# itz-sayak/C-Users-Sayakdutta-Self-Supervised-Arbitrary-Scale-Point-Cloud-Upsampling-via-SNN

Hardware: AMD Instinct MI355X
Metric: upsampled query-points/sec (kNN + fn fwd + rotate + fd fwd + displace), 4x scale, M=48 T=4 (higher is better)
Workload: dtype f32 (GEMMs as 3 x f16 MFMA with f32 accumulation; outer kNN f64); 1 GPU; synthetic sphere N=5000 (seed 0), B=4096 grid queries per GPU per step, M=48, T=4, fn k=[24,18,12] emb 640, fd k=32 scales [8,16,32,48] emb 768, conditioned-random weights seed 0, in-patch kNN recomputed every batch; cloud_points=5000, neighbours=48, outer_knn=f64 brute force, parallelism=query shards x1

## Files before the change

c-users-sayakdutta-self-supervised-arbitrary-scale-point-cloud-upsampling-via-snn_amd/_lib.py:

```python
import ctypes
import os
from ctypes import POINTER, c_char_p, c_double, c_float, c_int, c_int32, c_int64, c_void_p

_HERE = os.path.dirname(os.path.abspath(__file__))
LIB_PATH = os.environ.get("SAPCU_LIB_PATH") or os.path.join(_HERE, "csrc", "libsapcu_hip.so")
EXACT_LIB_PATH = os.path.join(_HERE, "csrc", "libsapcu_hip_exact.so")

FN_TAPS = ("stem", "block1", "block2", "block3", "pooled", "enc", "logits")
FD_TAPS = ("fused0", "spikes", "knn", "pooled", "enc", "x0")
KIND_FN, KIND_FD = 0, 1
ABI_VERSION = 2


class SapcuLibraryError(RuntimeError):
    """The HIP library is absent or unloadable (never silently replaced by a CPU path)."""


class SapcuError(RuntimeError):
    """A C entry point returned a non-zero status: args = (code, text)."""


_SIGNATURES = {
    "sapcu_abi_version": (c_int, []),
    "sapcu_last_error": (c_char_p, []),
    "sapcu_knn_gather_f64": (c_int, [c_void_p, c_int64, c_void_p, c_int64, c_int, c_void_p, c_void_p, c_void_p, c_void_p]),
    "sapcu_gather_rotate_f64": (c_int, [c_void_p, c_int64, c_void_p, c_int64, c_void_p, c_int, c_void_p, c_void_p, c_void_p]),
    "sapcu_displace_f64": (c_int, [c_void_p, c_void_p, c_void_p, c_int64, c_void_p, c_void_p]),
    "sapcu_knn_grid_workspace_bytes": (c_int64, [c_int64]),
    "sapcu_knn_self_grid_f64": (c_int, [c_void_p, c_int64, c_int64, c_int64, c_int, c_double, c_void_p, c_void_p, c_void_p, c_int64,
                                        POINTER(c_int64), c_void_p]),
    "sapcu_outlier_stats_f64": (c_int, [c_void_p, c_int64, c_int, c_int64, c_void_p, c_void_p, c_void_p]),
    "sapcu_outlier_keep_f64": (c_int, [c_void_p, c_int64, c_double, c_double, c_void_p, c_void_p]),
    "sapcu_fps_workspace_bytes": (c_int64, [c_int64]),
    "sapcu_fps_f32": (c_int, [c_void_p, c_int64, c_int64, c_void_p, c_void_p, c_int64, c_void_p]),
    "sapcu_dense_seeds_host": (c_int, [c_void_p, c_int64, c_double, c_void_p, c_int64, POINTER(c_int64)]),
    "sapcu_lif_train_forward": (c_int, [c_void_p, c_int64, c_int, c_int] + [c_void_p] * 4 + [c_void_p, c_void_p]),
    "sapcu_lif_train_workspace_bytes": (c_int64, [c_int64, c_int]),
    "sapcu_lif_train_backward": (c_int, [c_void_p, c_void_p, c_int64, c_int, c_int] + [c_void_p] * 4 + [c_void_p] * 5 +
                                 [c_void_p, c_int64, c_void_p]),
    "sapcu_train_workspace_bytes": (c_int64, [c_int64, c_int, c_int]),
    "sapcu_bn_train_forward": (c_int, [c_void_p, c_int64, c_int, c_void_p, c_void_p, c_float] + [c_void_p] * 4 + [c_void_p, c_int64, c_void_p]),
    "sapcu_bn_train_backward": (c_int, [c_void_p, c_void_p, c_int64, c_int] + [c_void_p] * 3 + [c_void_p] * 3 + [c_void_p, c_int64, c_void_p]),
    "sapcu_conv1x1_wgrad_f32": (c_int, [c_void_p, c_int, c_void_p, c_int, c_int64, c_int, c_int, c_void_p, c_void_p, c_void_p, c_int64, c_void_p]),
    "sapcu_gemm_bf16": (c_int, [c_void_p, c_int64, c_int, c_int, c_void_p, c_int, c_void_p, c_void_p, c_int, c_void_p]),
    "sapcu_wgrad_bf16_workspace_bytes": (c_int64, [c_int64, c_int, c_int]),
    "sapcu_conv1x1_wgrad_bf16": (c_int, [c_void_p, c_int, c_void_p, c_int, c_int64, c_int, c_int, c_void_p, c_void_p, c_void_p, c_int64, c_void_p]),
    "sapcu_softmax_agg_forward": (c_int, [c_void_p, c_void_p, c_void_p, c_int, c_void_p, c_void_p, c_int64, c_int, c_int, c_int, c_float, c_void_p, c_void_p]),
    "sapcu_softmax_agg_backward": (c_int, [c_void_p, c_void_p, c_void_p, c_int, c_void_p, c_void_p, c_void_p, c_int64, c_int, c_int, c_int, c_float,
                                          c_void_p, c_void_p, c_void_p, c_int, c_void_p]),
    "sapcu_gather_rows": (c_int, [c_void_p, c_int, c_void_p, c_int64, c_int, c_void_p, c_void_p]),
    "sapcu_scatter_add_rows": (c_int, [c_void_p, c_void_p, c_int64, c_int, c_void_p, c_int, c_int64, c_void_p]),
    "sapcu_scatter_add_rows_grouped": (c_int, [c_void_p, c_void_p, c_int64, c_int, c_void_p, c_int, c_int64, c_int, c_int, c_void_p, c_void_p]),
    "sapcu_group_max_forward": (c_int, [c_void_p, c_int64, c_int, c_int, c_void_p, c_void_p, c_void_p]),
    "sapcu_group_max_backward": (c_int, [c_void_p, c_void_p, c_int64, c_int, c_int, c_void_p, c_void_p]),
    "sapcu_neuron_selfloop": (c_int, [c_void_p, c_int64, c_int, c_int] + [c_void_p] * 6 + [c_void_p] * 4 + [c_void_p]),
    "sapcu_neuron_drive": (c_int, [c_void_p, c_int64, c_int, c_int] + [c_void_p] * 6 + [c_int] + [c_void_p] * 5 + [c_void_p]),
    "sapcu_patch_knn": (c_int, [c_void_p, c_int64, c_int, c_int, c_int, c_int, c_void_p, c_void_p]),
    "sapcu_model_create": (c_int, [c_int, POINTER(c_int32), c_int, c_void_p, c_int64, POINTER(c_int64), c_int,
                                   POINTER(c_void_p)]),
    "sapcu_model_destroy": (c_int, [c_void_p]),
    "sapcu_workspace_bytes": (c_int64, [c_void_p, c_int64, c_int]),
    "sapcu_model_gate_violations": (c_int, [c_void_p, POINTER(c_int)]),
    "sapcu_l2_normalize3": (c_int, [c_void_p, c_void_p, c_int64, c_void_p]),
    "sapcu_fn_forward": (c_int, [c_void_p, c_void_p, c_int64, c_int, c_void_p, c_void_p, c_void_p, c_void_p, c_int64,
                                 POINTER(c_void_p), c_void_p]),
    "sapcu_fd_forward": (c_int, [c_void_p, c_void_p, c_int64, c_int, c_void_p, c_void_p, c_void_p, c_int64,
                                 POINTER(c_void_p), c_void_p]),
    "sapcu_gemm_f32": (c_int, [c_void_p, c_int64, c_int, c_int, c_void_p, c_int, c_void_p, c_void_p, c_int, c_void_p,
                               c_int, c_void_p, c_int, c_int, c_void_p]),
    "sapcu_to_split_rows": (c_int, [c_void_p, c_int64, c_int, c_int, c_void_p, c_int, c_void_p]),
    "sapcu_posenc_gemm_f32": (c_int, [c_void_p, c_int64, c_int, c_void_p, c_void_p, c_void_p, c_int, c_void_p, c_void_p,
                                      c_int, c_int, c_void_p, c_void_p, c_void_p, c_void_p, c_int, c_void_p]),
    "sapcu_model_gemm_mode": (c_int, [c_void_p, POINTER(c_int), POINTER(c_int)]),
    "sapcu_model_fused_blocks": (c_int, [c_void_p, c_int, POINTER(c_int)]),
    "sapcu_fn_edge_chain_workspace_bytes": (c_int64, [c_int64, c_int, c_int]),
    "sapcu_fn_edge_chain_f32": (c_int, [c_void_p, c_void_p, c_int64, c_int, c_int, c_int] + [c_void_p] * 12 + [c_int, c_int, c_void_p, c_void_p,
                                        c_int64, c_void_p]),
}

EXPORTS = tuple(_SIGNATURES)

_SEEDS_SIGNATURES = {
    "sapcu_dense_seeds_workspace_bytes": (c_int64, [c_int64, c_int64]),
    "sapcu_dense_seeds_f64": (c_int, [c_void_p, c_int64, c_double, c_void_p, c_int64, c_int64, POINTER(c_int64), POINTER(c_int64),
                              c_void_p, c_int64, c_void_p]),
}
SEEDS_EXPORTS = tuple(_SEEDS_SIGNATURES)

_INTERNAL_SIGNATURES = {
    "sapcu_internal_fold_affine_host": (c_int, [c_void_p, c_void_p, c_void_p, c_void_p, c_int, c_int, c_void_p, c_void_p]),
}
_lib = None


def load(path=None):
    global _lib
    if _lib is not None and path is None:
        return _lib
    p = path or LIB_PATH
    if not os.path.exists(p):
        raise SapcuLibraryError(
            "HIP library not built: %s is missing. Run `make -C %s` (needs hipcc, gfx950). "
            "There is no CPU fallback." % (p, os.path.dirname(p)))
    try:
        lib = ctypes.CDLL(p)
    except OSError as e:
        raise SapcuLibraryError("cannot load %s: %s" % (p, e)) from e
    for name, (res, args) in list(_SIGNATURES.items()) + list(_SEEDS_SIGNATURES.items()) + list(_INTERNAL_SIGNATURES.items()):
        try:
            fn = getattr(lib, name)
        except AttributeError as e:
            raise SapcuLibraryError("%s does not export %s" % (p, name)) from e
        fn.restype = res
        fn.argtypes = args
    if lib.sapcu_abi_version() != ABI_VERSION:
        raise SapcuLibraryError("ABI version mismatch: library %d, binding %d" % (lib.sapcu_abi_version(), ABI_VERSION))
    if path is None:
        _lib = lib
    return lib


def check(rc):
    if rc != 0:
        text = load().sapcu_last_error()
        raise SapcuError(int(rc), text.decode("utf-8", "replace") if text else "")


def ptr(t):
    return None if t is None else c_void_p(t.data_ptr())


def current_stream():
    import torch
    return c_void_p(torch.cuda.current_stream().cuda_stream)
```

c-users-sayakdutta-self-supervised-arbitrary-scale-point-cloud-upsampling-via-snn_amd/csrc/gemm_epi.h:

```cpp
#pragma once
#include "common.h"

namespace sapcu {

typedef float f32x16 __attribute__((ext_vector_type(16)));

typedef _Float16 epi_half8 __attribute__((ext_vector_type(8)));
typedef float epi_f32x4 __attribute__((ext_vector_type(4)));
__device__ __forceinline__ f32x16 mfma_32x32x16_f16(epi_half8 a, epi_half8 b, f32x16 c) {
#ifdef SAPCU_TIMING_MFMA16
    epi_f32x4 q0 = {c[0], c[1], c[2], c[3]}, q1 = {c[8], c[9], c[10], c[11]};
    q0 = __builtin_amdgcn_mfma_f32_16x16x32_f16(a, b, q0, 0, 0, 0);
    q1 = __builtin_amdgcn_mfma_f32_16x16x32_f16(a, b, q1, 0, 0, 0);
    c[0] = q0[0]; c[1] = q0[1]; c[2] = q0[2]; c[3] = q0[3];
    c[8] = q1[0]; c[9] = q1[1]; c[10] = q1[2]; c[11] = q1[3];
    return c;
#else
    return __builtin_amdgcn_mfma_f32_32x32x16_f16(a, b, c, 0, 0, 0);
#endif
}

__device__ __forceinline__ float4 ld4(const float* p) { return *reinterpret_cast<const float4*>(p); }

__device__ __forceinline__ void lds_barrier() { asm volatile("s_waitcnt lgkmcnt(0)\n\ts_barrier" ::: "memory"); }

__device__ __forceinline__ float settle(float x) {
    asm volatile("" : "+v"(x));
    return x;
}

__device__ __forceinline__ void settle4(float4& v) { asm volatile("" : "+v"(v.x), "+v"(v.y), "+v"(v.z), "+v"(v.w)); }

__device__ __forceinline__ bool split_interleaved(int ld) { return (ld & 31) == 0; }
__device__ __forceinline__ int split_hi_index(int ld, int col) { return split_interleaved(ld) ? ((col >> 5) << 6) + (col & 31) : col; }
__device__ __forceinline__ int split_lo_index(int ld, int col) { return split_interleaved(ld) ? ((col >> 5) << 6) + 32 + (col & 31) : ld + col; }

__device__ __forceinline__ void store_split(float* base, int64_t row, int ld, int col, float v) {
    _Float16* rp = reinterpret_cast<_Float16*>(base + row * ld);
    const _Float16 hi = (_Float16)v;
    rp[split_hi_index(ld, col)] = hi;
    rp[split_lo_index(ld, col)] = (_Float16)(v - (float)hi);
}

template <int EPI, int W>
__device__ __forceinline__ void epilogue_group(const GemmArgs& g, const float (&acc)[W], int64_t row, int col,
                                               float bias, const NeuronP& np, const float (&q)[W],
                                               const float (&kf)[W]) {
    float v[W], res[W];
    bool ok[W];
#pragma unroll
    for (int u = 0; u < W; ++u) ok[u] = (row + u) < g.r;
    if (EPI == EPI_RESID || EPI == EPI_RESID_GELU) {
#pragma unroll
        for (int u = 0; u < W; ++u) res[u] = ok[u] ? g.resid[(row + u) * g.ldr + col] : 0.f;
    }
#pragma unroll
    for (int u = 0; u < W; ++u) v[u] = __fadd_rn(acc[u], bias);
    if (EPI == EPI_LIF || EPI == EPI_LIF_ATTN || EPI == EPI_LIF_MAX) lif_selfloop_n<W>(v, np, g.lif_T);
#pragma unroll
    for (int u = 0; u < W; ++u) {
        if (EPI == EPI_GELU) v[u] = gelu_erf(v[u]);
        if (EPI == EPI_LRELU || EPI == EPI_LRELU_MAX) v[u] = lrelu02(v[u]);
        if (EPI == EPI_RESID) v[u] = __fadd_rn(v[u], res[u]);
        if (EPI == EPI_RESID_GELU) v[u] = gelu_erf(__fadd_rn(v[u], res[u]));
    }
    if (EPI == EPI_LRELU_MAX || EPI == EPI_LIF_MAX) {
        int64_t cur = -1;
        float best = 0.f;
#pragma unroll
        for (int u = 0; u < W; ++u) {
            if (!ok[u]) continue;
            const int64_t grp = (row + u) / g.max_m;
            if (grp != cur) {
                if (cur >= 0) atomicMax(g.max_keys + cur * g.n + col, float_max_key(best));
                cur = grp;
                best = v[u];
            } else {
                best = fmaxf(best, v[u]);
            }
        }
        if (cur >= 0) atomicMax(g.max_keys + cur * g.n + col, float_max_key(best));
        return;
    }
#pragma unroll
    for (int u = 0; u < W; ++u) {
        if (!ok[u]) continue;
        if (g.c_split) {
            store_split(g.c, row + u, g.ldc, col, v[u]);
            if (EPI != EPI_LIF && EPI != EPI_LIF_ATTN && !(fabsf(v[u]) < 65504.0f) && g.ovf) atomicAdd(g.ovf, 1);
        } else {
            g.c[(row + u) * g.ldc + col] = v[u];
        }
        if (EPI == EPI_LIF_ATTN) {
            const float ai = __fadd_rn(__fsub_rn(q[u], kf[u]), v[u]);
            if (g.c2_split) store_split(g.c2, row + u, g.ldc, col, ai);
            else g.c2[(row + u) * g.ldc + col] = ai;
        }
    }
}

struct ColParams4 {
    float4 bias;
    float4 decay, adapt, rdecay, theta0;
};

template <bool VEC>
__device__ __forceinline__ float4 ld4_cols(const float* p, int col, int n) {
    if (VEC) return ld4(p + col);
    float4 r;
    r.x = col < n ? p[col] : 0.f;
    r.y = col + 1 < n ? p[col + 1] : 0.f;
    r.z = col + 2 < n ? p[col + 2] : 0.f;
    r.w = col + 3 < n ? p[col + 3] : 0.f;
    return r;
}

template <int EPI, bool VEC>
__device__ __forceinline__ ColParams4 load_col_params4(const GemmArgs& g, int col, bool valid) {
    ColParams4 c;
    const float4 z = make_float4(0.f, 0.f, 0.f, 0.f);
    c.bias = (valid && g.bias) ? ld4_cols<VEC>(g.bias, col, g.n) : z;
    c.decay = c.adapt = c.rdecay = c.theta0 = z;
    if (EPI == EPI_LIF || EPI == EPI_LIF_ATTN) {
        const int cc = valid ? col : 0;
        c.decay = ld4_cols<VEC>(g.lif, cc, g.n);
        c.adapt = ld4_cols<VEC>(g.lif + g.n, cc, g.n);
        c.rdecay = ld4_cols<VEC>(g.lif + 2 * (int64_t)g.n, cc, g.n);
        c.theta0 = ld4_cols<VEC>(g.lif + 3 * (int64_t)g.n, cc, g.n);
    }
    return c;
}

__device__ __forceinline__ void clamp_col_params4(const ColParams4& c, NeuronP2 (&np)[2]) {
    np[0].decay = f32x2{clampf(c.decay.x, 0.1f, 0.99f), clampf(c.decay.y, 0.1f, 0.99f)};
    np[1].decay = f32x2{clampf(c.decay.z, 0.1f, 0.99f), clampf(c.decay.w, 0.1f, 0.99f)};
    np[0].adapt = f32x2{clampf(c.adapt.x, 0.001f, 0.1f), clampf(c.adapt.y, 0.001f, 0.1f)};
    np[1].adapt = f32x2{clampf(c.adapt.z, 0.001f, 0.1f), clampf(c.adapt.w, 0.001f, 0.1f)};
    np[0].rdecay = f32x2{clampf(c.rdecay.x, 0.1f, 0.95f), clampf(c.rdecay.y, 0.1f, 0.95f)};
    np[1].rdecay = f32x2{clampf(c.rdecay.z, 0.1f, 0.95f), clampf(c.rdecay.w, 0.1f, 0.95f)};
    np[0].theta0 = f32x2{c.theta0.x, c.theta0.y};
    np[1].theta0 = f32x2{c.theta0.z, c.theta0.w};
}

typedef _Float16 half4 __attribute__((ext_vector_type(4)));

template <bool VEC>
__device__ __forceinline__ void store_f32x4(float* base, int64_t row, int ld, int col, int n, const float (&v)[4]) {
    if (VEC) {
        *reinterpret_cast<float4*>(base + row * ld + col) = make_float4(v[0], v[1], v[2], v[3]);
    } else {
#pragma unroll
        for (int u = 0; u < 4; ++u)
            if (col + u < n) base[row * ld + col + u] = v[u];
    }
}

template <bool VEC>
__device__ __forceinline__ void store_split4(float* base, int64_t row, int ld, int col, int n, const float (&v)[4]) {
    if (!VEC) {
#pragma unroll
        for (int u = 0; u < 4; ++u)
            if (col + u < n) store_split(base, row, ld, col + u, v[u]);
        return;
    }
    _Float16* rp = reinterpret_cast<_Float16*>(base + row * ld);
    half4 hi, lo;
#pragma unroll
    for (int u = 0; u < 4; ++u) {
        hi[u] = (_Float16)v[u];
        lo[u] = (_Float16)(v[u] - (float)hi[u]);
    }
    *reinterpret_cast<half4*>(rp + split_hi_index(ld, col)) = hi;
    *reinterpret_cast<half4*>(rp + split_lo_index(ld, col)) = lo;
}

template <int EPI, bool VEC>
__device__ __forceinline__ void epilogue_row4_compute(const GemmArgs& g, const float4 acc, int64_t row, int col,
                                                      const ColParams4& cp, float (&v)[4]) {
    v[0] = __fmaf_rn(acc.x, 0.0625f, cp.bias.x);
    v[1] = __fmaf_rn(acc.y, 0.0625f, cp.bias.y);
    v[2] = __fmaf_rn(acc.z, 0.0625f, cp.bias.z);
    v[3] = __fmaf_rn(acc.w, 0.0625f, cp.bias.w);
    float4 res = make_float4(0.f, 0.f, 0.f, 0.f);
    if (EPI == EPI_RESID || EPI == EPI_RESID_GELU) res = ld4_cols<VEC>(g.resid + row * g.ldr, col, g.n);
    if (EPI == EPI_LIF || EPI == EPI_LIF_ATTN) {
        f32x2 pv[2] = {f32x2{v[0], v[1]}, f32x2{v[2], v[3]}};
        NeuronP2 np[2];
        clamp_col_params4(cp, np);
        lif_selfloop_pairs<2>(pv, np, g.lif_T);
        v[0] = pv[0].x; v[1] = pv[0].y; v[2] = pv[1].x; v[3] = pv[1].y;
    }
    const float rs[4] = {res.x, res.y, res.z, res.w};
#pragma unroll
    for (int u = 0; u < 4; ++u) {
        if (EPI == EPI_GELU) v[u] = gelu_erf(v[u]);
        if (EPI == EPI_LRELU) v[u] = lrelu02(v[u]);
        if (EPI == EPI_RESID) v[u] = __fadd_rn(v[u], rs[u]);
        if (EPI == EPI_RESID_GELU) v[u] = gelu_erf(__fadd_rn(v[u], rs[u]));
    }
}

template <int EPI, bool VEC>
__device__ __forceinline__ void epilogue_row4_store(const GemmArgs& g, const float (&v)[4], int64_t row, int col,
                                                    const float4 q, const float4 kf) {
    float ai[4] = {0.f, 0.f, 0.f, 0.f};
    if (EPI == EPI_LIF_ATTN) {
        ai[0] = __fadd_rn(__fsub_rn(q.x, kf.x), v[0]);
        ai[1] = __fadd_rn(__fsub_rn(q.y, kf.y), v[1]);
        ai[2] = __fadd_rn(__fsub_rn(q.z, kf.z), v[2]);
        ai[3] = __fadd_rn(__fsub_rn(q.w, kf.w), v[3]);
        asm volatile("" : "+v"(ai[0]), "+v"(ai[1]), "+v"(ai[2]), "+v"(ai[3])::"memory");
    }
    if (g.c_split) {
        store_split4<VEC>(g.c, row, g.ldc, col, g.n, v);
        if (EPI != EPI_LIF && EPI != EPI_LIF_ATTN && g.ovf) {
            float big = 0.f;
#pragma unroll
            for (int u = 0; u < 4; ++u)
                if (VEC || col + u < g.n) big = fmaxf(big, fabsf(v[u]));
            const bool nan = (VEC || col < g.n) && !(v[0] == v[0] && v[1] == v[1] && v[2] == v[2] && v[3] == v[3]);
            if (!(big < 65504.0f) || nan) atomicAdd(g.ovf, 1);
        }
    } else {
        store_f32x4<VEC>(g.c, row, g.ldc, col, g.n, v);
    }
    if (EPI == EPI_LIF_ATTN) {
        if (g.c2_split) store_split4<VEC>(g.c2, row, g.ldc, col, g.n, ai);
        else store_f32x4<VEC>(g.c2, row, g.ldc, col, g.n, ai);
    }
}

template <int EPI>
__device__ __forceinline__ void epilogue_group4(const GemmArgs& g, const float (&acc)[4], int64_t row, int col,
                                                float bias, const NeuronP& np, const float (&q)[4],
                                                const float (&kf)[4]) {
    epilogue_group<EPI, 4>(g, acc, row, col, bias, np, q, kf);
}

}
```

c-users-sayakdutta-self-supervised-arbitrary-scale-point-cloud-upsampling-via-snn_amd/csrc/gemm_f32.hip:

```cpp
#include "common.h"
#include "gemm_epi.h"

namespace sapcu {

constexpr int BM = 128, BN = 128, BK = 32, LDT = BK + 4;
constexpr int OPER_FLOATS = 2 * (BM + BN) * LDT;
constexpr int STAGE_FLOATS = 4 * 64 * 64;
constexpr int LDS_BYTES = (OPER_FLOATS + STAGE_FLOATS) * 4;

template <int EPI>
__global__ __launch_bounds__(512, 2) void gemm_kernel(const GemmArgs g) {
    extern __shared__ __attribute__((aligned(16))) float smem[];
    float* stage = smem + OPER_FLOATS;
    const int tid = threadIdx.x;
    const int lane = tid & 63, wave = tid >> 6;
    const bool producer = wave < 4;
    const int pw = wave & 3;
    const int wm = pw >> 1, wn = pw & 1;
    const int r32 = lane & 31, h = lane >> 5;

    const int ntn = (g.n + BN - 1) / BN;
    const int64_t ntm = (g.r + BM - 1) / BM;
    const int64_t ntiles = ntm * ntn;
    const int nx = gridDim.x < 8 ? 1 : 8;
// ... 57 lines not shown
            for (int i = 0; i < 4; ++i) {
                *reinterpret_cast<float4*>(&sA[(srow + 32 * i) * LDT + skc]) = ra[i];
                *reinterpret_cast<float4*>(&sW[(srow + 32 * i) * LDT + skc]) = rw[i];
            }
        };

        const bool cons_work = !producer && prev_row0 >= 0;
        float cbias[2];
        NeuronP cnp[2];
        bool ccol[2];
        if (cons_work) {
#pragma unroll
            for (int j = 0; j < 2; ++j) {
                const int col = prev_col0 + wn * 64 + j * 32 + r32;
                ccol[j] = col < g.n;
                cbias[j] = settle((ccol[j] && g.bias) ? g.bias[col] : 0.f);
                if (EPI == EPI_LIF || EPI == EPI_LIF_ATTN) {
                    cnp[j] = load_lif(g.lif, g.n, ccol[j] ? col : 0);
                    cnp[j].theta0 = settle(cnp[j].theta0);
                }
            }
        }
        const int gper = (16 + nk - 1) / nk;
        int2 tabrow = make_int2(0, 0);
        float nq[4] = {0.f, 0.f, 0.f, 0.f}, nkf[4] = {0.f, 0.f, 0.f, 0.f};
        auto issue_gather = [&](int gi) {
            if (EPI != EPI_LIF_ATTN) return;
            const int t4 = gi >> 2, e4 = gi & 3;
            const int i = t4 >> 1, j = t4 & 1;
            const int col = prev_col0 + wn * 64 + j * 32 + r32;
            const int lrow = i * 32 + 8 * e4 + 4 * h;
#pragma unroll
            for (int u = 0; u < 4; ++u) {
                const int qr = __shfl(tabrow.x, lrow + u);
                const int kr = __shfl(tabrow.y, lrow + u);
                const bool ok = col < g.n && (prev_row0 + wm * 64 + lrow + u) < g.r;
                nq[u] = ok ? g.q[(int64_t)qr * g.ldq + col] : 0.f;
                nkf[u] = ok ? g.kf[(int64_t)kr * g.ldq + col] : 0.f;
            }
        };
        if (cons_work && EPI == EPI_LIF_ATTN) {
            const int64_t trow = prev_row0 + wm * 64 + lane;
            if (trow < g.r) tabrow = g.tab[trow];
            tabrow.x = __builtin_bit_cast(int, settle(__builtin_bit_cast(float, tabrow.x)));
            tabrow.y = __builtin_bit_cast(int, settle(__builtin_bit_cast(float, tabrow.y)));
            issue_gather(0);
        }
        auto consume = [&](int s) {
            if (!cons_work) return;
            for (int gi = s * gper; gi < (s + 1) * gper && gi < 16; ++gi) {
                const int t4 = gi >> 2, e4 = gi & 3;
                const int i = t4 >> 1, j = t4 & 1;
                float cq[4], ckf[4];
#pragma unroll
                for (int u = 0; u < 4; ++u) {
                    cq[u] = nq[u];
                    ckf[u] = nkf[u];
                }
                if (gi + 1 < 16) issue_gather(gi + 1);
                if (!(j ? ccol[1] : ccol[0])) continue;
                const int64_t row = prev_row0 + wm * 64 + i * 32 + 8 * e4 + 4 * h;
                if (row >= g.r) continue;
                float a[4];
#pragma unroll
                for (int u = 0; u < 4; ++u) a[u] = stage[(pw * 64 + gi * 4 + u) * 64 + lane];
                NeuronP np;
                np.decay = j ? cnp[1].decay : cnp[0].decay;
                np.adapt = j ? cnp[1].adapt : cnp[0].adapt;
                np.rdecay = j ? cnp[1].rdecay : cnp[0].rdecay;
                np.theta0 = j ? cnp[1].theta0 : cnp[0].theta0;
                np.dT = 0.f;
                np.rh = 0.f;
                epilogue_group4<EPI>(g, a, row, prev_col0 + wn * 64 + j * 32 + r32, j ? cbias[1] : cbias[0], np, cq, ckf);
            }
        };

        if (producer && have) {
            load_tile(0);
            store_tile(0);
        }
        lds_barrier();
        int cur = 0;
        for (int kt = 0; kt < nk; ++kt) {
            if (producer) {
                if (have) {
                    if (kt + 1 < nk) load_tile((kt + 1) * BK);
                    const float* sA = smem + cur * (BM + BN) * LDT + (wm * 64 + r32) * LDT + h * 4;
                    const float* sW = smem + cur * (BM + BN) * LDT + BM * LDT + (wn * 64 + r32) * LDT + h * 4;
                    float4 fa[2][2], fb[2][2];
                    fa[0][0] = ld4(sA);
                    fa[0][1] = ld4(sA + 32 * LDT);
                    fb[0][0] = ld4(sW);
                    fb[0][1] = ld4(sW + 32 * LDT);
#pragma unroll
                    for (int k8 = 0; k8 < BK / 8; ++k8) {
                        const int cb = k8 & 1, nb = cb ^ 1;
                        if (k8 + 1 < BK / 8) {
                            fa[nb][0] = ld4(sA + (k8 + 1) * 8);
                            fa[nb][1] = ld4(sA + 32 * LDT + (k8 + 1) * 8);
                            fb[nb][0] = ld4(sW + (k8 + 1) * 8);
                            fb[nb][1] = ld4(sW + 32 * LDT + (k8 + 1) * 8);
                        }
                        const float av[2][4] = {{fa[cb][0].x, fa[cb][0].y, fa[cb][0].z, fa[cb][0].w},
                                                {fa[cb][1].x, fa[cb][1].y, fa[cb][1].z, fa[cb][1].w}};
                        const float bv[2][4] = {{fb[cb][0].x, fb[cb][0].y, fb[cb][0].z, fb[cb][0].w},
                                                {fb[cb][1].x, fb[cb][1].y, fb[cb][1].z, fb[cb][1].w}};
#pragma unroll
                        for (int e = 0; e < 4; ++e)
#pragma unroll
                            for (int i = 0; i < 2; ++i)
#pragma unroll
                                for (int j = 0; j < 2; ++j)
                                    acc[i][j] = __builtin_amdgcn_mfma_f32_32x32x2f32(av[i][e], bv[j][e], acc[i][j], 0, 0, 0);
                    }
                    if (kt + 1 < nk) store_tile(cur ^ 1);
                }
            } else {
                consume(kt);
            }
            lds_barrier();
            cur ^= 1;
        }
        if (producer && have) {
#pragma unroll
            for (int i = 0; i < 2; ++i)
#pragma unroll
                for (int j = 0; j < 2; ++j)
#pragma unroll
                    for (int e = 0; e < 16; ++e) stage[(pw * 64 + (i * 2 + j) * 16 + e) * 64 + lane] = acc[i][j][e];
        }
        lds_barrier();
        prev_row0 = have ? row0 : -1;
        prev_col0 = col0;
    }
}

template <int EPI>
static int launch_t(const GemmArgs& g, hipStream_t st) {
    static DeviceOnce lds_once;
    SAPCU_SET_MAX_LDS(lds_once, (&gemm_kernel<EPI>), LDS_BYTES);
    const int g_num_cus = device_cu_count();
    const int64_t tiles = ((g.r + BM - 1) / BM) * ((g.n + BN - 1) / BN);
    const int64_t grid = tiles < g_num_cus ? tiles : g_num_cus;
    hipLaunchKernelGGL((gemm_kernel<EPI>), dim3((unsigned)grid), dim3(512), LDS_BYTES, st, g);
    SAPCU_CHECK_LAUNCH();
    return SAPCU_OK;
}

int launch_gemm(const GemmArgs& g, hipStream_t st) {
    if (g.r == 0 || g.n == 0) return SAPCU_OK;
    SAPCU_CHECK_ARG(g.k > 0 && g.k % BK == 0, "gemm: k=%d must be a positive multiple of %d", g.k, BK);
    SAPCU_CHECK_ARG(g.lda % 4 == 0 && ((uintptr_t)g.a & 15) == 0 && ((uintptr_t)g.w & 15) == 0,
                    "gemm: A/W must be 16-byte aligned with lda %% 4 == 0 (lda=%d)", g.lda);
    switch (g.epi) {
        case EPI_BIAS: return launch_t<EPI_BIAS>(g, st);
        case EPI_LIF: return launch_t<EPI_LIF>(g, st);
        case EPI_GELU: return launch_t<EPI_GELU>(g, st);
        case EPI_RESID: return launch_t<EPI_RESID>(g, st);
        case EPI_LRELU: return launch_t<EPI_LRELU>(g, st);
        case EPI_RESID_GELU: return launch_t<EPI_RESID_GELU>(g, st);
        case EPI_LIF_ATTN:
            SAPCU_CHECK_ARG(g.ldq > 0 && g.tab && g.q && g.kf && g.c2, "gemm: bad attn operands");
            return launch_t<EPI_LIF_ATTN>(g, st);
        default: set_error("gemm: unknown epilogue %d", g.epi); return SAPCU_ERR_ARG;
    }
}

}
```

c-users-sayakdutta-self-supervised-arbitrary-scale-point-cloud-upsampling-via-snn_amd/csrc/gemm_sf16.hip:

```cpp
#include "common.h"
#include "gemm_epi.h"

namespace sapcu {

typedef _Float16 half8 __attribute__((ext_vector_type(8)));
typedef __attribute__((address_space(3))) unsigned char lds_byte;
typedef const __attribute__((address_space(1))) void* gptr_t;

constexpr int SBM = 128, SBN = 128, SBK = 64;
constexpr int PLANE_BYTES = SBM * SBK * 2;
constexpr int STAGE_BYTES = 4 * PLANE_BYTES;
constexpr int HALF_HANDOFF_BYTES = 8 * 16 * 64 * 4;
constexpr int SF16_LDS_BYTES = 2 * STAGE_BYTES + HALF_HANDOFF_BYTES;

__device__ __forceinline__ void split8(const float4& x0, const float4& x1, half8& hi, half8& lo, float& amax) {
    const float xs[8] = {x0.x, x0.y, x0.z, x0.w, x1.x, x1.y, x1.z, x1.w};
#pragma unroll
    for (int i = 0; i < 8; ++i) {
        const _Float16 h = (_Float16)xs[i];
        hi[i] = h;
        lo[i] = (_Float16)(xs[i] - (float)h);
        amax = fmaxf(amax, fabsf(xs[i]));
    }
}
// ... 134 lines not shown
                            __builtin_amdgcn_sched_barrier(0);
                        };
                        product(1, 0);
                        product(0, 1);
                        product(0, 0);
                    }
                    if (kt + 1 < nk) {
                        store_a(cur ^ 1);
                        asm volatile("s_waitcnt vmcnt(0)" ::: "memory");
                    }
                }
                lds_barrier();
                cur ^= 1;
            }
            if (have) {
#pragma unroll
                for (int e = 0; e < 16; ++e) {
                    stage0[(pw * 16 + e) * 64 + lane] = __fmul_rn(acc[0][e], 0.0625f);
                    stage1[(pw * 16 + e) * 64 + lane] = __fmul_rn(acc[1][e], 0.0625f);
                }
                if (amax > 65504.0f && g.ovf) atomicAdd(g.ovf, 1);
            }
            lds_barrier();
            prev = have;
        }
    } else {
        int64_t prev_row0 = -1;
        int prev_col0 = 0;
        const int gper = (8 + nk - 1) / nk;
        for (int64_t it = 0;; ++it) {
            const int64_t local = it * wgs_per_x + wg_in_x;
            const bool have = local < x_count;
            if (!have && prev_row0 < 0) break;
            const int64_t logical = x_begin + local;
            const bool cons_work = prev_row0 >= 0;
            float cacc[16];
#pragma unroll
            for (int q = 0; q < 16; ++q) cacc[q] = cons_work ? stage1[(pw * 16 + q) * 64 + lane] : 0.f;
            float cbias[2];
            NeuronP cnp[2];
            bool ccol[2];
#pragma unroll
            for (int j = 0; j < 2; ++j) {
                const int col = prev_col0 + wn * 64 + j * 32 + r32;
                ccol[j] = cons_work && col < g.n;
                cbias[j] = settle((ccol[j] && g.bias) ? g.bias[col] : 0.f);
                cnp[j] = NeuronP{0.f, 0.f, 0.f, 0.f, 0.f, 0.f};
                if (EPI == EPI_LIF || EPI == EPI_LIF_ATTN || EPI == EPI_LIF_MAX) {
                    cnp[j] = load_lif(g.lif, g.n, ccol[j] ? col : 0);
                    cnp[j].theta0 = settle(cnp[j].theta0);
                }
            }
            int2 tabrow = make_int2(0, 0);
            float nq[4] = {0.f, 0.f, 0.f, 0.f}, nkf[4] = {0.f, 0.f, 0.f, 0.f};
            auto issue_gather = [&](int gi) {
                if (EPI != EPI_LIF_ATTN) return;
                const int j = gi >> 2, e4 = gi & 3;
                const int col = prev_col0 + wn * 64 + j * 32 + r32;
                const int lrow = 8 * e4 + 4 * h;
#pragma unroll
                for (int u = 0; u < 4; ++u) {
                    const int qr = __shfl(tabrow.x, lrow + u);
                    const int kr = __shfl(tabrow.y, lrow + u);
                    const bool ok = col < g.n && (prev_row0 + wm * 32 + lrow + u) < g.r;
                    nq[u] = ok ? g.q[(int64_t)qr * g.ldq + col] : 0.f;
                    nkf[u] = ok ? g.kf[(int64_t)kr * g.ldq + col] : 0.f;
                }
            };
            if (cons_work && EPI == EPI_LIF_ATTN) {
                const int64_t trow = prev_row0 + wm * 32 + (lane & 31);
                if (trow < g.r) tabrow = g.tab[trow];
                tabrow.x = __builtin_bit_cast(int, settle(__builtin_bit_cast(float, tabrow.x)));
                tabrow.y = __builtin_bit_cast(int, settle(__builtin_bit_cast(float, tabrow.y)));
                issue_gather(0);
            }
            lds_barrier();
            for (int kt = 0; kt < nk; ++kt) {
                if (cons_work) {
                    for (int gi = kt * gper; gi < (kt + 1) * gper && gi < 8; ++gi) {
                        float cq[4], ckf[4];
#pragma unroll
                        for (int u = 0; u < 4; ++u) {
                            cq[u] = nq[u];
                            ckf[u] = nkf[u];
                        }
                        if (gi + 1 < 8) issue_gather(gi + 1);
                        const int j = gi >> 2, e4 = gi & 3;
                        if (!(j ? ccol[1] : ccol[0])) continue;
                        const int64_t row = prev_row0 + wm * 32 + 8 * e4 + 4 * h;
                        if (row >= g.r) continue;
                        const int col = prev_col0 + wn * 64 + j * 32 + r32;
                        if (gi < 4) {
                            float a[4];
#pragma unroll
                            for (int u = 0; u < 4; ++u) a[u] = stage0[(pw * 16 + gi * 4 + u) * 64 + lane];
                            epilogue_group4<EPI>(g, a, row, col, cbias[0], cnp[0], cq, ckf);
                        } else {
                            switch (gi) {
                                case 4: consume_reg_group<EPI, 0>(g, cacc, row, col, cbias[1], cnp[1], cq, ckf); break;
                                case 5: consume_reg_group<EPI, 1>(g, cacc, row, col, cbias[1], cnp[1], cq, ckf); break;
                                case 6: consume_reg_group<EPI, 2>(g, cacc, row, col, cbias[1], cnp[1], cq, ckf); break;
                                default: consume_reg_group<EPI, 3>(g, cacc, row, col, cbias[1], cnp[1], cq, ckf); break;
                            }
                        }
                    }
                }
                lds_barrier();
            }
            lds_barrier();
            prev_row0 = have ? (logical / ntn) * SBM : -1;
            prev_col0 = have ? (int)(logical % ntn) * SBN : 0;
        }
    }
}

__global__ __launch_bounds__(256) void split_weights_kernel(const float* __restrict__ w, int64_t count,
                                                            _Float16* __restrict__ hi, _Float16* __restrict__ lo,
                                                            int* __restrict__ ovf) {
    const int64_t t = (int64_t)blockIdx.x * blockDim.x + threadIdx.x;
    if (t >= count) return;
    const float x = w[t] * 16.0f;
    const _Float16 hh = (_Float16)x;
    hi[t] = hh;
    lo[t] = (_Float16)(x - (float)hh);
    if (!(fabsf(x) < 65504.0f)) atomicAdd(ovf, 1);
}

int launch_split_weights(const float* w, int64_t count, void* hi, void* lo, int* ovf, hipStream_t st) {
    if (count == 0) return SAPCU_OK;
    hipLaunchKernelGGL(split_weights_kernel, dim3((unsigned)((count + 255) / 256)), dim3(256), 0, st, w, count,
                       (_Float16*)hi, (_Float16*)lo, ovf);
    SAPCU_CHECK_LAUNCH();
    return SAPCU_OK;
}

template <int EPI>
static int launch_t16(const GemmArgs& g, hipStream_t st) {
    static DeviceOnce lds_once;
    SAPCU_SET_MAX_LDS(lds_once, (&gemm_sf16_kernel<EPI>), SF16_LDS_BYTES);
    const int g_num_cus16 = device_cu_count();
    const int64_t tiles = ((g.r + SBM - 1) / SBM) * ((g.n + SBN - 1) / SBN);
    const int64_t grid = tiles < g_num_cus16 ? tiles : g_num_cus16;
    hipLaunchKernelGGL((gemm_sf16_kernel<EPI>), dim3((unsigned)grid), dim3(1024), SF16_LDS_BYTES, st, g);
    SAPCU_CHECK_LAUNCH();
    return SAPCU_OK;
}

int launch_gemm_sf16(const GemmArgs& g, hipStream_t st) {
    if (g.r == 0 || g.n == 0) return SAPCU_OK;
    SAPCU_CHECK_ARG(g.k > 0 && g.k % SBK == 0, "gemm_sf16: k=%d must be a positive multiple of %d", g.k, SBK);
    SAPCU_CHECK_ARG(g.lda % 4 == 0 && ((uintptr_t)g.a & 15) == 0 && g.w16_hi && g.w16_lo &&
                        ((uintptr_t)g.w16_hi & 15) == 0 && ((uintptr_t)g.w16_lo & 15) == 0,
                    "gemm_sf16: operands must be 16-byte aligned (lda=%d)", g.lda);
    switch (g.epi) {
        case EPI_BIAS: return launch_t16<EPI_BIAS>(g, st);
        case EPI_LIF: return launch_t16<EPI_LIF>(g, st);
        case EPI_GELU: return launch_t16<EPI_GELU>(g, st);
        case EPI_RESID: return launch_t16<EPI_RESID>(g, st);
        case EPI_LRELU: return launch_t16<EPI_LRELU>(g, st);
        case EPI_LRELU_MAX:
            SAPCU_CHECK_ARG(g.max_keys && g.max_m >= 1, "gemm_sf16: EPI_LRELU_MAX needs max_keys and max_m");
            return launch_t16<EPI_LRELU_MAX>(g, st);
        case EPI_LIF_MAX:
            SAPCU_CHECK_ARG(g.max_keys && g.max_m >= 1 && g.lif, "gemm_sf16: EPI_LIF_MAX needs max_keys, max_m and neuron parameters");
            return launch_t16<EPI_LIF_MAX>(g, st);
        case EPI_RESID_GELU: return launch_t16<EPI_RESID_GELU>(g, st);
        case EPI_LIF_ATTN:
            SAPCU_CHECK_ARG(g.ldq > 0 && g.tab && g.q && g.kf && g.c2, "gemm_sf16: bad attn operands");
            return launch_t16<EPI_LIF_ATTN>(g, st);
        default: set_error("gemm_sf16: unknown epilogue %d", g.epi); return SAPCU_ERR_ARG;
    }
}

}
```

c-users-sayakdutta-self-supervised-arbitrary-scale-point-cloud-upsampling-via-snn_amd/csrc/gemm_sf16_bt.hip:

```cpp
#include "common.h"
#include "gemm_epi.h"

namespace sapcu {

typedef _Float16 half8 __attribute__((ext_vector_type(8)));
typedef __attribute__((address_space(3))) unsigned char lds_byte;
typedef const __attribute__((address_space(1))) void* gptr_t;

constexpr int TBM = 256, TBK = 32;
constexpr int TA_PLANE = TBM * TBK * 2;
constexpr int TA_SLOT = 2 * TA_PLANE;
constexpr int TA_SLOTS = 3;
constexpr int TW_SLOTS = 2;

template <int N>
__device__ __forceinline__ void bt_wait_vm() {
    if (N == 16) asm volatile("s_waitcnt vmcnt(16)" ::: "memory");
    else if (N == 8) asm volatile("s_waitcnt vmcnt(8)" ::: "memory");
    else if (N == 4) asm volatile("s_waitcnt vmcnt(4)" ::: "memory");
    else asm volatile("s_waitcnt vmcnt(0)" ::: "memory");
}

__device__ __forceinline__ float bt_load_f32(const float* p) {
    float v;
// ... 124 lines not shown
    const int kstep_bytes = a_il ? 128 : TBK * 2;
    const char* const op_base = is_a ? reinterpret_cast<const char*>(g.a) : reinterpret_cast<const char*>(g.w16_hi);
    const int pieces = is_a ? 4 : W_PIECES;
    const int rows_per_wave = 16 * pieces;
    const int depth = is_a ? TA_SLOTS : TW_SLOTS;
    const int slot_bytes = is_a ? TA_SLOT : W_SLOT;
    const int plane_bytes = is_a ? TA_PLANE : W_PLANE;
    const int64_t total_steps = my_tiles * nk;
    int64_t pf_tile = 0, pf_tm = first_tm;
    int pf_kt = 0, pf_tn = first_tn;
    const char* pf_base = nullptr;
    unsigned pf_off[4] = {0, 0, 0, 0};
    const int lrow = rows_per_wave * sub + (lane >> 2);
    auto pf_setup = [&]() {
        const int64_t first = is_a ? pf_tm * TBM : (int64_t)pf_tn * BN;
        const int64_t left = (is_a ? g.r : (int64_t)g.n) - first;
        pf_base = op_base + first * pitch_b;
#pragma unroll
        for (int p = 0; p < 4; ++p) {
            int rr = lrow + 16 * p;
            if (rr >= left) rr = (int)(left - 1);
            pf_off[p] = (unsigned)(rr * (int)pitch_b + dsb);
        }
    };
    lds_byte* const ring0 = (lds_byte*)(smem_raw + (is_a ? 0 : A_BYTES) + sub * rows_per_wave * 64);
    int issue_slot = 0;
    int64_t issued = 0;
    auto issue = [&]() {
        lds_byte* sb = ring0 + issue_slot * slot_bytes;
        const char* src = pf_base + pf_kt * kstep_bytes;
#pragma unroll
        for (int p = 0; p < 4; ++p) {
            if (p < pieces) {
                __builtin_amdgcn_global_load_lds((gptr_t)(src + pf_off[p]), sb + p * 1024, 16, 0, 0);
                __builtin_amdgcn_global_load_lds((gptr_t)(src + lo_delta + pf_off[p]), sb + plane_bytes + p * 1024, 16, 0, 0);
            }
        }
        ++issued;
        if (++issue_slot == depth) issue_slot = 0;
        if (++pf_kt == nk) {
            pf_kt = 0;
            ++pf_tile;
            pf_tm += step_tm;
            pf_tn += step_tn;
            if (pf_tn >= ntn) { pf_tn -= ntn; ++pf_tm; }
            if (pf_tile < my_tiles) pf_setup();
        }
    };
    pf_setup();
    while (issued < depth && issued < total_steps) issue();
    int64_t landed_upto = 0;
    auto wait_landed = [&](int64_t step) {
        if (step < landed_upto) return;
        const int64_t ahead = issued - step - 1;
        if (is_a) {
            if (ahead >= 2) bt_wait_vm<16>();
            else if (ahead == 1) bt_wait_vm<8>();
            else bt_wait_vm<0>();
        } else if (W_PIECES == 4) {
            if (ahead >= 1) bt_wait_vm<8>();
            else bt_wait_vm<0>();
        } else {
            if (ahead >= 1) bt_wait_vm<4>();
            else bt_wait_vm<0>();
        }
    };

    constexpr int CS = 2 * CT;
    const int c16 = lane & 15, g4 = lane >> 4;
    const unsigned frag_ko = (unsigned)((g4 ^ ((c16 >> 2) & 3)) * 16);
    const unsigned a_frag0 = (unsigned)((wm * 128 + c16) * (TBK * 2)) + frag_ko;
    const unsigned w_frag0 = (unsigned)(A_BYTES + (wn * 32 * CT + c16) * (TBK * 2)) + frag_ko;
    half8 ah0[4], al0[4], ah1[4], al1[4], wh[CS], wl[CS];
    auto read_a = [&](int a_slot, int half, half8 (&ah)[4], half8 (&al)[4]) {
        const unsigned char* sA = smem_raw + a_slot * TA_SLOT + a_frag0 + half * 4 * 16 * (TBK * 2);
#pragma unroll
        for (int i = 0; i < 4; ++i) {
            ah[i] = *reinterpret_cast<const half8*>(sA + i * 16 * (TBK * 2));
            al[i] = *reinterpret_cast<const half8*>(sA + i * 16 * (TBK * 2) + TA_PLANE);
        }
    };
    auto read_w = [&](int w_slot, int chalf) {
        const unsigned char* sW = smem_raw + w_slot * W_SLOT + w_frag0;
#pragma unroll
        for (int j = chalf * CT; j < (chalf + 1) * CT; ++j) {
            wh[j] = *reinterpret_cast<const half8*>(sW + j * 16 * (TBK * 2));
            wl[j] = *reinterpret_cast<const half8*>(sW + j * 16 * (TBK * 2) + W_PLANE);
        }
    };
    f32x4 acc[8][CS];
    auto mfma_group = [&](int rhalf, const half8 (&ah)[4], const half8 (&al)[4], int chalf) {
#pragma unroll
        for (int i = 0; i < 4; ++i)
#pragma unroll
            for (int j = chalf * CT; j < (chalf + 1) * CT; ++j)
                acc[4 * rhalf + i][j] = __builtin_amdgcn_mfma_f32_16x16x32_f16(al[i], wh[j], acc[4 * rhalf + i][j], 0, 0, 0);
#pragma unroll
        for (int i = 0; i < 4; ++i)
#pragma unroll
            for (int j = chalf * CT; j < (chalf + 1) * CT; ++j)
                acc[4 * rhalf + i][j] = __builtin_amdgcn_mfma_f32_16x16x32_f16(ah[i], wl[j], acc[4 * rhalf + i][j], 0, 0, 0);
#pragma unroll
        for (int i = 0; i < 4; ++i)
#pragma unroll
            for (int j = chalf * CT; j < (chalf + 1) * CT; ++j)
                acc[4 * rhalf + i][j] = __builtin_amdgcn_mfma_f32_16x16x32_f16(ah[i], wh[j], acc[4 * rhalf + i][j], 0, 0, 0);
    };

    wait_landed(0);
    lds_barrier();
    int ca = 0, cw = 0, na = 1, nw = 1;
    int64_t gstep = 0;
    int64_t tm = first_tm;
    int tn = first_tn;
    for (int64_t ti = 0; ti < my_tiles; ++ti) {
#pragma unroll
        for (int i = 0; i < 8; ++i)
#pragma unroll
            for (int j = 0; j < CS; ++j) acc[i][j] = f32x4{0.f, 0.f, 0.f, 0.f};
        read_w(cw, 0);
        read_w(cw, 1);
        read_a(ca, 0, ah0, al0);
        for (int kt = 0; kt < nk; ++kt, ++gstep) {
            read_a(ca, 1, ah1, al1);
            mfma_group(0, ah0, al0, 0);
            mfma_group(0, ah0, al0, 1);
            const bool more = kt + 1 < nk;
            if (gstep + 1 < total_steps) {
                wait_landed(gstep + 1);
                lds_barrier();
                if (issued < total_steps && !(is_a && kt + 1 == nk)) issue();
                if (more) read_a(na, 0, ah0, al0);
            } else {
                lds_barrier();
            }
            mfma_group(1, ah1, al1, 0);
            if (more) read_w(nw, 0);
            mfma_group(1, ah1, al1, 1);
            if (more) read_w(nw, 1);
            ca = na;
            cw = nw;
            if (++na == TA_SLOTS) na = 0;
            if (++nw == TW_SLOTS) nw = 0;
        }
        const int64_t row0 = tm * TBM + wm * 128;
        const int col0 = tn * BN + wn * 32 * CT;
        float pbias[CS], praw[CS][4];
        NeuronP pnp[CS];
#pragma unroll
        for (int j = 0; j < CS; ++j) {
            const int col = col0 + j * 16 + c16;
            pbias[j] = 0.f;
            if (g.bias) pbias[j] = bt_load_f32(g.bias + col);
            if (EPI == EPI_LIF || EPI == EPI_LIF_ATTN) {
#pragma unroll
                for (int q = 0; q < 4; ++q) praw[j][q] = bt_load_f32(g.lif + (int64_t)q * g.n + col);
            }
        }
        bt_wait_vm<0>();
        landed_upto = issued;
        if (is_a && issued < total_steps) issue();
        __builtin_amdgcn_sched_barrier(0);
#pragma unroll
        for (int j = 0; j < CS; ++j) {
            pnp[j] = NeuronP{0.f, 0.f, 0.f, 0.f, 0.f, 0.f};
            if (EPI == EPI_LIF || EPI == EPI_LIF_ATTN) {
                pnp[j].decay = clampf(praw[j][0], 0.1f, 0.99f);
                pnp[j].adapt = clampf(praw[j][1], 0.001f, 0.1f);
                pnp[j].rdecay = clampf(praw[j][2], 0.1f, 0.95f);
                pnp[j].theta0 = praw[j][3];
            }
        }
        const bool interior = tm * TBM + TBM <= g.r;
        if (EPI == EPI_LRELU_MAX) {
#pragma unroll
            for (int j = 0; j < CS; ++j) {
                const int col = col0 + j * 16 + c16;
                int64_t cur = -1, boundary = 0;
                float best = 0.f;
#pragma unroll
                for (int rs = 0; rs < 8; ++rs) {
#pragma unroll
                    for (int e = 0; e < 4; ++e) {
                        const int64_t rr = row0 + rs * 16 + 4 * g4 + e;
                        if (rr >= g.r) continue;
                        const float v = lrelu02(__fadd_rn(__fmul_rn(acc[rs][j][e], 0.0625f), pbias[j]));
                        if (rr >= boundary) {
                            if (cur >= 0) atomicMax(g.max_keys + cur * g.n + col, float_max_key(best));
                            cur = rr / g.max_m;
                            boundary = (cur + 1) * g.max_m;
                            best = v;
                        } else {
                            best = fmaxf(best, v);
                        }
                    }
                }
                if (cur >= 0) atomicMax(g.max_keys + cur * g.n + col, float_max_key(best));
            }
        } else if (interior && EPI == EPI_LIF_ATTN && !g.c_split && g.c2_split) {
            bt_epilogue_fast<EPI, CS, false, true>(g, acc, row0, col0, c16, g4, pbias, pnp);
        } else if (interior && EPI == EPI_LIF && g.c_split) {
            bt_epilogue_fast<EPI, CS, true, false>(g, acc, row0, col0, c16, g4, pbias, pnp);
        } else if (interior && EPI != EPI_LIF_ATTN && !g.c_split) {
            bt_epilogue_fast<EPI, CS, false, false>(g, acc, row0, col0, c16, g4, pbias, pnp);
        } else
#pragma unroll
        for (int rs = 0; rs < 8; ++rs) {
            const int64_t row = row0 + rs * 16 + 4 * g4;
            if (row >= g.r) continue;
            int2 t4[4];
            if (EPI == EPI_LIF_ATTN) {
#pragma unroll
                for (int u = 0; u < 4; ++u) t4[u] = row + u < g.r ? g.tab[row + u] : make_int2(0, 0);
            }
#pragma unroll
            for (int j = 0; j < CS; ++j) {
                const int col = col0 + j * 16 + c16;
                float a4[4], cq[4] = {0.f, 0.f, 0.f, 0.f}, ckf[4] = {0.f, 0.f, 0.f, 0.f};
#pragma unroll
                for (int u = 0; u < 4; ++u) a4[u] = __fmul_rn(acc[rs][j][u], 0.0625f);
                if (EPI == EPI_LIF_ATTN) {
#pragma unroll
                    for (int u = 0; u < 4; ++u) {
                        cq[u] = g.q[(int64_t)t4[u].x * g.ldq + col];
                        ckf[u] = g.kf[(int64_t)t4[u].y * g.ldq + col];
                    }
                }
                epilogue_group4<EPI>(g, a4, row, col, pbias[j], pnp[j], cq, ckf);
            }
            __builtin_amdgcn_sched_barrier(0);
        }
        tm += step_tm;
        tn += step_tn;
        if (tn >= ntn) { tn -= ntn; ++tm; }
    }
}

template <int EPI, int BN>
static int launch_bt_t(const GemmArgs& g, hipStream_t st) {
    constexpr int LDS = TA_SLOTS * TA_SLOT + TW_SLOTS * 2 * BN * TBK * 2;
    static DeviceOnce lds_once;
    SAPCU_SET_MAX_LDS(lds_once, (&gemm_bt_kernel<EPI, BN>), LDS);
    const int g_num_cus_bt = device_cu_count();
    const int64_t tiles = ((g.r + TBM - 1) / TBM) * (g.n / BN);
    const int64_t grid = tiles < g_num_cus_bt ? tiles : g_num_cus_bt;
    hipLaunchKernelGGL((gemm_bt_kernel<EPI, BN>), dim3((unsigned)grid), dim3(512), LDS, st, g);
    SAPCU_CHECK_LAUNCH();
    return SAPCU_OK;
}

bool gemm_sf16_bt_ok(const GemmArgs& g) {
    if (!g.a_split || !g.w16_hi || !g.w16_lo || g.k <= 0 || g.k % TBK || g.k > g.lda || g.lda % 8) return false;
    if (((uintptr_t)g.a & 15) || ((uintptr_t)g.w16_hi & 15) || ((uintptr_t)g.w16_lo & 15)) return false;
    if (g.n % 128) return false;
    if (4 * (int64_t)g.lda * TBM >= (1LL << 31)) return false;
    if (g.r < 4 * TBM) return false;
    auto al16 = [](const void* p) { return ((uintptr_t)p & 15) == 0; };
    if (g.ldc % 4 || !al16(g.c) || (g.bias && !al16(g.bias))) return false;
    if ((g.epi == EPI_LIF || g.epi == EPI_LIF_ATTN) && !al16(g.lif)) return false;
    if (g.epi == EPI_LIF_ATTN && (g.ldq % 4 || !al16(g.q) || !al16(g.kf) || !al16(g.c2))) return false;
    if (g.epi == EPI_LRELU_MAX) return g.max_keys != nullptr && g.max_m >= 1;
    return g.epi == EPI_BIAS || g.epi == EPI_LIF || g.epi == EPI_LIF_ATTN;
}

int launch_gemm_sf16_bt(const GemmArgs& g, hipStream_t st) {
    if (g.r == 0 || g.n == 0) return SAPCU_OK;
    SAPCU_CHECK_ARG(gemm_sf16_bt_ok(g), "gemm_bt: unsupported shape or epilogue");
    if (g.epi == EPI_LIF || g.epi == EPI_LIF_ATTN) SAPCU_CHECK_ARG(g.lif, "gemm_bt: missing neuron parameters");
    if (g.epi == EPI_LIF_ATTN) SAPCU_CHECK_ARG(g.ldq > 0 && g.tab && g.q && g.kf && g.c2, "gemm_bt: bad attn operands");
    const bool wide = g.n % 256 == 0;
    switch (g.epi) {
        case EPI_LRELU_MAX: return wide ? launch_bt_t<EPI_LRELU_MAX, 256>(g, st) : launch_bt_t<EPI_LRELU_MAX, 128>(g, st);
        case EPI_BIAS: return wide ? launch_bt_t<EPI_BIAS, 256>(g, st) : launch_bt_t<EPI_BIAS, 128>(g, st);
        case EPI_LIF: return wide ? launch_bt_t<EPI_LIF, 256>(g, st) : launch_bt_t<EPI_LIF, 128>(g, st);
        default: return wide ? launch_bt_t<EPI_LIF_ATTN, 256>(g, st) : launch_bt_t<EPI_LIF_ATTN, 128>(g, st);
    }
}


}
```

c-users-sayakdutta-self-supervised-arbitrary-scale-point-cloud-upsampling-via-snn_amd/csrc/gemm_sf16_ring.hip:

```cpp
#include "common.h"
#include "gemm_epi.h"

namespace sapcu {

typedef _Float16 half8 __attribute__((ext_vector_type(8)));
typedef __attribute__((address_space(3))) unsigned char lds_byte;
typedef const __attribute__((address_space(1))) void* gptr_t;

constexpr int RBM = 128, RBN = 128, RBK = 32;
constexpr bool RING_TILES_INTERLEAVED = true;
constexpr int RPLANE = RBM * RBK * 2;
constexpr int ROPSLOT = 2 * RPLANE;
constexpr int RING_SLOTS = 8;
constexpr int RING_BYTES = RING_SLOTS * ROPSLOT;
constexpr int RHAND = 8 * 16 * 64 * 4;
constexpr int RING_LDS_BYTES = RING_BYTES + RHAND;

template <int N>
__device__ __forceinline__ void wait_vm() {
    if (N >= 16) asm volatile("s_waitcnt vmcnt(16)" ::: "memory");
    else if (N == 12) asm volatile("s_waitcnt vmcnt(12)" ::: "memory");
    else if (N == 8) asm volatile("s_waitcnt vmcnt(8)" ::: "memory");
    else if (N == 4) asm volatile("s_waitcnt vmcnt(4)" ::: "memory");
    else asm volatile("s_waitcnt vmcnt(0)" ::: "memory");
// ... 165 lines not shown
                    acc[0] = mfma_32x32x16_f16(f1.al, f1.wh[0], acc[0]);
                    acc[1] = mfma_32x32x16_f16(f1.al, f1.wh[1], acc[1]);
                    acc[0] = mfma_32x32x16_f16(f0.ah, f0.wl[0], acc[0]);
                    acc[1] = mfma_32x32x16_f16(f0.ah, f0.wl[1], acc[1]);
                    acc[0] = mfma_32x32x16_f16(f1.ah, f1.wl[0], acc[0]);
                    acc[1] = mfma_32x32x16_f16(f1.ah, f1.wl[1], acc[1]);
                    acc[0] = mfma_32x32x16_f16(f0.ah, f0.wh[0], acc[0]);
                    acc[1] = mfma_32x32x16_f16(f0.ah, f0.wh[1], acc[1]);
                    acc[0] = mfma_32x32x16_f16(f1.ah, f1.wh[0], acc[0]);
                    acc[1] = mfma_32x32x16_f16(f1.ah, f1.wh[1], acc[1]);
                    if (gstep + 1 < total_steps) {
                        wait_landed(gstep + 1);
                        lds_barrier();
                        if (issued < total_steps) issue();
                        read_frags(na, nw, 0, f0);
                    } else {
                        lds_barrier();
                    }
                    ca = na;
                    cw = nw;
                    if (++na == RA_SLOTS) na = 0;
                    if (++nw == RW_SLOTS) nw = 0;
                    continue;
                }
                mfma6(f0);
                if (gstep + 1 < total_steps) {
                    wait_landed(gstep + 1);
                    lds_barrier();
                    if (issued < total_steps) issue();
                    read_frags(na, nw, 0, f0);
                } else {
                    lds_barrier();
                }
                mfma6(f1);
                ca = na;
                cw = nw;
                if (++na == RA_SLOTS) na = 0;
                if (++nw == RW_SLOTS) nw = 0;
            }
#pragma unroll
            for (int jj = 0; jj < 2; ++jj) {
                const int j = 1 - jj;
                lds_barrier();
#pragma unroll
                for (int e = 0; e < 16; ++e) {
                    float* hb = (e & 1) ? hand_odd : hand_even;
                    hb[((e & 3) + 8 * (e >> 2)) * 32] = acc[j][e];
                }
                lds_barrier();
            }
        }
    } else {
        const int c4 = lane & 7, rs = lane >> 3;
        auto hand_at = [&](int p) -> const float4* {
            const int rr = p * 8 + rs;
            return reinterpret_cast<const float4*>(hand + pw * 1024 + (rr ^ ((rr >> 2) & 1)) * 32 + c4 * 4);
        };
        float4 cacc[4];
        int64_t prev_row0 = -1;
        int prev_col0 = 0;
        int64_t cur_tm = first_tm;
        int cur_tn = first_tn;
        const int pper = (8 + nk - 1) / nk;
        lds_barrier();
        for (int64_t ti = 0; ti <= my_tiles; ++ti) {
            const bool have = ti < my_tiles;
            const bool cons_work = prev_row0 >= 0;
            bool ccol[2];
#pragma unroll
            for (int j = 0; j < 2; ++j) ccol[j] = cons_work && (prev_col0 + wn * 64 + j * 32 + c4 * 4) < g.n;
            ColParams4 cp;
            cp.bias = cp.decay = cp.adapt = cp.rdecay = cp.theta0 = make_float4(0.f, 0.f, 0.f, 0.f);
            int2 tabrow = make_int2(0, 0);
            if (cons_work && EPI == EPI_LIF_ATTN) {
                const int64_t trow = prev_row0 + wm * 32 + (lane & 31);
                if (trow < g.r) tabrow = g.tab[trow];
                tabrow.x = __builtin_bit_cast(int, settle(__builtin_bit_cast(float, tabrow.x)));
                tabrow.y = __builtin_bit_cast(int, settle(__builtin_bit_cast(float, tabrow.y)));
            }
            for (int kt = 0; kt < nk; ++kt) {
                if (cons_work)
                for (int pi = kt * pper; pi < (kt + 1) * pper && pi < 8; ++pi) {
                    const int j = pi >> 2, p4 = pi & 3, rr = p4 * 8 + rs;
                    const int64_t row = prev_row0 + wm * 32 + rr;
                    const int col = prev_col0 + wn * 64 + j * 32 + c4 * 4;
                    const bool active = (j ? ccol[1] : ccol[0]) && row < g.r;
                    if (p4 == 0) {
                        cp = load_col_params4<EPI, VEC>(g, col, j ? ccol[1] : ccol[0]);
                        settle4(cp.bias);
                        if (EPI == EPI_LIF || EPI == EPI_LIF_ATTN) {
                            settle4(cp.decay);
                            settle4(cp.adapt);
                            settle4(cp.rdecay);
                            settle4(cp.theta0);
                        }
                    }
                    float4 cq = make_float4(0.f, 0.f, 0.f, 0.f), ckf = cq;
                    if (EPI == EPI_LIF_ATTN) {
                        const int qr = __shfl(tabrow.x, rr);
                        const int kr = __shfl(tabrow.y, rr);
                        if (active) {
                            cq = ld4_cols<VEC>(g.q + (int64_t)qr * g.ldq, col, g.n);
                            ckf = ld4_cols<VEC>(g.kf + (int64_t)kr * g.ldq, col, g.n);
                        }
                    }
                    if (!active) continue;
                    float4 a;
                    if (j == 0) a = *hand_at(p4);
                    else switch (p4) {
                        case 0: a = cacc[0]; break;
                        case 1: a = cacc[1]; break;
                        case 2: a = cacc[2]; break;
                        default: a = cacc[3]; break;
                    }
                    float v[4];
                    epilogue_row4_compute<EPI, VEC>(g, a, row, col, cp, v);
                    epilogue_row4_store<EPI, VEC>(g, v, row, col, cq, ckf);
                }
                if (have) lds_barrier();
            }
            if (!have) break;
            lds_barrier();
            lds_barrier();
#pragma unroll
            for (int p = 0; p < 4; ++p) cacc[p] = *hand_at(p);
            lds_barrier();
            lds_barrier();
            prev_row0 = cur_tm * RBM;
            prev_col0 = cur_tn * RBN;
            cur_tm += step_tm;
            cur_tn += step_tn;
            if (cur_tn >= ntn) { cur_tn -= ntn; ++cur_tm; }
        }
    }
}

template <int EPI, bool VEC, bool PM = false>
static int launch_ring_tv(const GemmArgs& g, hipStream_t st) {
    static DeviceOnce lds_once;
    SAPCU_SET_MAX_LDS(lds_once, (&gemm_ring_kernel<EPI, VEC, PM>), RING_LDS_BYTES);
    const int g_num_cus_ring = device_cu_count();
    const int row_step = RBM;
    const int64_t tiles = ((g.r + row_step - 1) / row_step) * ((g.n + RBN - 1) / RBN);
    const int64_t grid = tiles < g_num_cus_ring ? tiles : g_num_cus_ring;
    hipLaunchKernelGGL((gemm_ring_kernel<EPI, VEC, PM>), dim3((unsigned)grid), dim3(1024), RING_LDS_BYTES, st, g);
    SAPCU_CHECK_LAUNCH();
    return SAPCU_OK;
}

static bool ring_vec_ok(const GemmArgs& g) {
    auto al16 = [](const void* p) { return ((uintptr_t)p & 15) == 0; };
    bool ok = g.n % 4 == 0 && g.ldc % 4 == 0 && al16(g.c) && (!g.bias || al16(g.bias));
    if (g.epi == EPI_LIF || g.epi == EPI_LIF_ATTN) ok = ok && al16(g.lif);
    if (g.epi == EPI_RESID || g.epi == EPI_RESID_GELU) ok = ok && g.ldr % 4 == 0 && al16(g.resid);
    if (g.epi == EPI_LIF_ATTN) ok = ok && g.ldq % 4 == 0 && al16(g.q) && al16(g.kf) && al16(g.c2);
    return ok;
}

template <int EPI>
static int launch_ring_t(const GemmArgs& g, hipStream_t st) {
    return ring_vec_ok(g) ? launch_ring_tv<EPI, true, true>(g, st) : launch_ring_tv<EPI, false, true>(g, st);
}
int launch_gemm_sf16_ring(const GemmArgs& g, hipStream_t st) {
    if (g.r == 0 || g.n == 0) return SAPCU_OK;
    SAPCU_CHECK_ARG(g.a_split, "gemm_ring: A must be in split rows");
    SAPCU_CHECK_ARG(g.k > 0 && g.k % RBK == 0 && g.k <= g.lda, "gemm_ring: k=%d must be a multiple of %d and <= lda", g.k, RBK);
    SAPCU_CHECK_ARG(g.lda % 8 == 0 && ((uintptr_t)g.a & 15) == 0 && g.w16_hi && g.w16_lo &&
                        ((uintptr_t)g.w16_hi & 15) == 0 && ((uintptr_t)g.w16_lo & 15) == 0,
                    "gemm_ring: operands must be 16-byte aligned with lda %% 8 == 0 (lda=%d)", g.lda);
    if (g.epi == EPI_LIF || g.epi == EPI_LIF_ATTN) SAPCU_CHECK_ARG(g.lif, "gemm_ring: missing neuron parameters");
    if (g.epi == EPI_RESID || g.epi == EPI_RESID_GELU) SAPCU_CHECK_ARG(g.resid, "gemm_ring: missing residual");
    switch (g.epi) {
        case EPI_BIAS: return launch_ring_t<EPI_BIAS>(g, st);
        case EPI_LIF: return launch_ring_t<EPI_LIF>(g, st);
        case EPI_GELU: return launch_ring_t<EPI_GELU>(g, st);
        case EPI_RESID: return launch_ring_t<EPI_RESID>(g, st);
        case EPI_LRELU: return launch_ring_t<EPI_LRELU>(g, st);
        case EPI_RESID_GELU: return launch_ring_t<EPI_RESID_GELU>(g, st);
        case EPI_LIF_ATTN:
            SAPCU_CHECK_ARG(g.ldq > 0 && g.tab && g.q && g.kf && g.c2, "gemm_ring: bad attn operands");
            return launch_ring_t<EPI_LIF_ATTN>(g, st);
        default: set_error("gemm_ring: unknown epilogue %d", g.epi); return SAPCU_ERR_ARG;
    }
}


}
```

c-users-sayakdutta-self-supervised-arbitrary-scale-point-cloud-upsampling-via-snn_amd/csrc/model.hip:

```cpp
#include <stdarg.h>
#include <stdlib.h>

#include <new>
#include <vector>

#include "common.h"
#include "ops.h"

namespace sapcu {

static thread_local char g_err[512] = "";

void set_error(const char* fmt, ...) {
    va_list ap;
    va_start(ap, fmt);
    vsnprintf(g_err, sizeof(g_err), fmt, ap);
    va_end(ap);
}

enum FnSlot {
    FN_STEM_W = 0, FN_STEM_B, FN_STEM_LIF,
    FN_BLK0 = 3,
    FN_FINAL_W = FN_BLK0 + 63, FN_FINAL_B, FN_FINAL_LIF,
    FN_FCOUT_W, FN_FCOUT_B,
    FN_MLP0_W, FN_MLP0_B, FN_MLP1_W, FN_MLP1_B, FN_MLP2_W, FN_MLP2_B,
    FN_HEAD_W, FN_HEAD_B, FN_LN_W, FN_LN_B,
    FN_SLOTS
};
enum FnBlkSlot {
    B_FC1_W = 0, B_FC1_B, B_SNN1,
    B_QKV_W, B_QKV_B, B_QKV_LIF,
    B_DELTA_W, B_DELTA_B, B_DELTA_LIF,
    B_DELTA2_W, B_DELTA2_B, B_DELTA2_LIF,
    B_GAMMA_W, B_GAMMA_B, B_GAMMA_LIF,
    B_GAMMA2_W, B_GAMMA2_B,
    B_OUT_W, B_OUT_B,
    B_FC2_W, B_FC2_B,
    B_SLOTS
};
static_assert(B_SLOTS == 21, "fn block slot count");
static_assert(FN_SLOTS == 81, "fn slot count");

enum FdSlot {
    FD_E0_W = 0, FD_E0_B,
    FD_FUSE_W, FD_FUSE_B, FD_SNN0,
    FD_EDGE1_W, FD_EDGE1_SHIFT, FD_SNN1,
    FD_EDGE2_W, FD_EDGE2_SHIFT, FD_SNN2,
    FD_EDGE3_W, FD_EDGE3_SHIFT, FD_SNN3,
    FD_MSC_W, FD_MSC_B,
    FD_TI_W, FD_SNNFC,
    FD_FCIN_W, FD_FCIN_B,
    FD_R0_FC0_W, FD_R0_FC0_B, FD_R0_FC4_W, FD_R0_FC4_B, FD_R0_PROJ_W, FD_R0_PROJ_B,
    FD_R1_FC0_W, FD_R1_FC0_B, FD_R1_FC4_W, FD_R1_FC4_B, FD_R1_PROJ_W, FD_R1_PROJ_B,
    FD_QKV_W, FD_QKV_B,
    FD_WO_T, FD_BO, FD_LN_W, FD_LN_B, FD_WH_T, FD_BH, FD_WD, FD_BD,
    FD_SLOTS
};
static_assert(FD_SLOTS == 42, "fd slot count");

}

struct sapcu_model {
    int kind;
    int kv[3];
    int k, nscale;
    int ks[8];
    int32_t* ks_dev;
    int* gate_dev;
    bool sf16;
    void* w16_hi;
    void* w16_lo;
    void* chain_w;
    int* ovf_dev;
    int emb, T, heads;
    int64_t chunk;
    int64_t ws_budget;
    bool opt_bt;
    bool opt_chain;
    bool opt_chain_wide;
    bool opt_fn_maxfuse;
    bool opt_fn_fold_out;
    bool opt_fd_maxfuse;
    bool opt_fd_split;
    bool opt_fd_fused;
    bool opt_fd_x0;
    void* fde_w;
    int64_t fde_off[5];
    float* fde_nprm;
    float* blob;
    int64_t blob_floats;
    int64_t fold_w[3], fold_b[3];
    std::vector<int64_t> dir;
    const float* p(int slot) const { return blob + dir[slot]; }
};

namespace sapcu {

struct Arena {
    char* base;
    int64_t cap, off;
    template <typename T>
    T* take(int64_t count) {
        const int64_t bytes = ((count * (int64_t)sizeof(T)) + 255) & ~(int64_t)255;
        T* p = reinterpret_cast<T*>(base + off);
        off += bytes;
        return p;
    }
};

static inline int64_t imax(int64_t a, int64_t b) { return a > b ? a : b; }
static inline int imin(int a, int b) { return a < b ? a : b; }

static bool split_rows_gemm_on_big_tile(const GemmArgs& g, bool allow_bt) { return allow_bt && gemm_sf16_bt_ok(g); }

int launch_gemm_split_rows(const GemmArgs& g, hipStream_t st, bool allow_bt) {
    if (split_rows_gemm_on_big_tile(g, allow_bt)) return launch_gemm_sf16_bt(g, st);
    return launch_gemm_sf16_ring(g, st);
}

static void fold_affine_f64(const float* w1, const float* b1, const float* w2, const float* b2, int d, int n, float* w_fold,
                            float* b_fold) {
    std::vector<double> acc((size_t)d);
    for (int i = 0; i < n; ++i) {
        for (int k = 0; k < d; ++k) acc[k] = 0.0;
        double bs = 0.0;
        for (int j = 0; j < d; ++j) {
            const double a = (double)w2[(int64_t)i * d + j];
            const float* row = w1 + (int64_t)j * d;
            for (int k = 0; k < d; ++k) acc[k] += a * (double)row[k];
            bs += a * (double)b1[j];
        }
        for (int k = 0; k < d; ++k) w_fold[(int64_t)i * d + k] = (float)acc[k];
        b_fold[i] = (float)(bs + (double)b2[i]);
    }
}

static bool env_off(const char* name) {
    const char* e = getenv(name);
    return e && strcmp(e, "0") == 0;
}

static int run_gemm(const sapcu_model* m, GemmArgs& g, hipStream_t st) {
    const bool have16 = m && m->sf16 && g.w >= m->blob && g.w < m->blob + m->blob_floats;
    if (have16) {
        const int64_t off = g.w - m->blob;
        g.w16_hi = (const _Float16*)m->w16_hi + off;
        g.w16_lo = (const _Float16*)m->w16_lo + off;
        g.ovf = m->ovf_dev;
        if (g.a_split) return launch_gemm_split_rows(g, st, m->opt_bt);
        if (g.k % 64 == 0) return launch_gemm_sf16(g, st);
    }
    if (g.a_split || g.c_split || g.c2_split) {
        set_error("run_gemm: split-row operands need the split-f16 kernels");
        return SAPCU_ERR_ARG;
    }
    return launch_gemm(g, st);
}

static int gemm(const sapcu_model* m, const float* a, int64_t r, int k, int lda, const float* w, int n,
                const float* bias, float* c, int ldc, int epi, hipStream_t st, const float* lif = nullptr,
                int lifT = 0, const float* resid = nullptr, int ldr = 0, int fmt = 0) {
    GemmArgs g;
    memset(&g, 0, sizeof(g));
    g.a = a; g.r = r; g.k = k; g.lda = lda; g.w = w; g.n = n; g.bias = bias; g.c = c; g.ldc = ldc;
    g.epi = epi; g.lif = lif; g.lif_T = lifT; g.resid = resid; g.ldr = ldr;
    g.a_split = fmt & 1; g.c_split = (fmt >> 1) & 1;
    return run_gemm(m, g, st);
}

#define SAPCU_TRY(expr)                 \
    do {                                \
        int _rc = (expr);               \
        if (_rc != SAPCU_OK) return _rc; \
    } while (0)

static int tap_copy(void* const* taps, int which, int64_t dst_off_bytes, const void* src, int64_t bytes,
                    hipStream_t st) {
    if (!taps || !taps[which] || bytes == 0) return SAPCU_OK;
    SAPCU_CHECK_HIP(hipMemcpyAsync((char*)taps[which] + dst_off_bytes, src, (size_t)bytes, hipMemcpyDeviceToDevice, st));
    return SAPCU_OK;
}

struct FnPlan {
    int64_t cb;
    int kk[3];
    int64_t edge_floats, edge_floats23;
};

static bool fn_block_fused(const sapcu_model* m, int l, int mp) {
    return m->sf16 && m->chain_w && m->opt_chain && fn_edge_chain_ok(128 << l, imin(m->kv[l], mp));
}

static void fn_edge_floats_per_patch(const sapcu_model* m, int mp, int64_t& first, int64_t& others) {
    first = (int64_t)mp * m->emb;
    others = 0;
    for (int l = 0; l < 3; ++l) {
        if (fn_block_fused(m, l, mp)) continue;
        const int64_t e = (int64_t)mp * imin(m->kv[l], mp) * (128 << l);
        first = imax(first, e);
        others = imax(others, e);
    }
}

static int64_t fn_bytes_per_patch(const sapcu_model* m, int mp) {
    int64_t e1, e23;
    fn_edge_floats_per_patch(m, mp, e1, e23);
    int kmx = 1;
    int64_t idxs = 0;
    for (int l = 0; l < 3; ++l) {
        const int kk = imin(m->kv[l], mp);
        idxs += (int64_t)mp * kk * 4;
        kmx = kmx > kk ? kmx : kk;
    }
    return (e1 + 2 * e23) * 4 + idxs + (int64_t)mp * kmx * 24 + (int64_t)mp * (64 + 192 + 512 + 1536 + 512) * 4 +
           ((int64_t)m->emb + 2048 + 1024 + 512 + 256 + 3) * 4;
}

static int64_t chunk_patches(const sapcu_model* m, int64_t b, int64_t bytes_per_patch) {
    int64_t cb = m->chunk;
    if (cb <= 0) {
        cb = m->ws_budget / (bytes_per_patch > 0 ? bytes_per_patch : 1);
        cb = cb < 64 ? 64 : (cb / 64) * 64;
    }
    if (cb > b) cb = b;
    return cb < 1 ? 1 : cb;
}

static FnPlan fn_plan(const sapcu_model* m, int64_t b, int mp) {
    FnPlan pl;
    pl.cb = chunk_patches(m, b, fn_bytes_per_patch(m, mp));
    for (int l = 0; l < 3; ++l) pl.kk[l] = imin(m->kv[l], mp);
    int64_t e1, e23;
    fn_edge_floats_per_patch(m, mp, e1, e23);
    pl.edge_floats = e1 * pl.cb;
    pl.edge_floats23 = e23 * pl.cb;
    return pl;
}

static int64_t fn_ws_bytes(const sapcu_model* m, int64_t b, int mp) {
    const FnPlan pl = fn_plan(m, b, mp);
    const int64_t P = pl.cb * mp;
    int64_t fl = 0;
    auto add = [&](int64_t n, int64_t esz) { fl += ((n * esz) + 255) & ~(int64_t)255; };
    for (int l = 0; l < 3; ++l) add(P * pl.kk[l], 4);
    { int kmx = 1; for (int l = 0; l < 3; ++l) kmx = kmx > pl.kk[l] ? kmx : pl.kk[l]; add(P * kmx, 8); add(P * kmx, 16); }
    add(P * 64, 4); add(P * 192, 4); add(P * 512, 4); add(P * 1536, 4); add(P * 512, 4);
    add(pl.edge_floats, 4); add(pl.edge_floats23, 4); add(pl.edge_floats23, 4);
    add(pl.cb * m->emb, 4); add(pl.cb * 2048, 4); add(pl.cb * 1024, 4); add(pl.cb * 512, 4); add(pl.cb * 256, 4);
    add(pl.cb * 3, 4);
    return fl + 256;
}

static int fn_forward(const sapcu_model* m, const float* patch, int64_t b, int mp, const int32_t* knn_in,
                      int32_t* knn_out, float* normals, void* ws, int64_t ws_bytes, void* const* taps,
                      hipStream_t st) {
    const FnPlan pl = fn_plan(m, b, mp);
    if (ws_bytes < fn_ws_bytes(m, b, mp)) {
        set_error("fn_forward: workspace %lld B < required %lld B", (long long)ws_bytes, (long long)fn_ws_bytes(m, b, mp));
        return SAPCU_ERR_WORKSPACE;
    }
    int64_t tab_off[3];
    tab_off[0] = 0;
    tab_off[1] = b * mp * pl.kk[0];
    tab_off[2] = tab_off[1] + b * mp * pl.kk[1];

    for (int64_t s = 0; s < b; s += pl.cb) {
        const int64_t cb = (b - s) < pl.cb ? (b - s) : pl.cb;
        const int64_t P = cb * mp;
        Arena A{(char*)(((uintptr_t)ws + 255) & ~(uintptr_t)255), ws_bytes, 0};
        int32_t* idx[3];
        for (int l = 0; l < 3; ++l) idx[l] = A.take<int32_t>(pl.cb * mp * pl.kk[l]);
        int kmx = 1;
        for (int l = 0; l < 3; ++l) kmx = kmx > pl.kk[l] ? kmx : pl.kk[l];
        int2* tab = A.take<int2>(pl.cb * mp * kmx);
        float4* pdiff = A.take<float4>(pl.cb * mp * kmx);
        float* feat0 = A.take<float>(pl.cb * mp * 64);
        float* cat = A.take<float>(pl.cb * mp * 192);
        float* X = A.take<float>(pl.cb * mp * 512);
        float* QKV = A.take<float>(pl.cb * mp * 1536);
        float* RES = A.take<float>(pl.cb * mp * 512);
        float* B1 = A.take<float>(pl.edge_floats);
        float* B2 = A.take<float>(pl.edge_floats23);
        float* B3 = A.take<float>(pl.edge_floats23);
        float* pooled = A.take<float>(pl.cb * m->emb);
        float* enc = A.take<float>(pl.cb * 2048);
        float* h1 = A.take<float>(pl.cb * 1024);
        float* h2 = A.take<float>(pl.cb * 512);
        float* h3 = A.take<float>(pl.cb * 256);
        float* logits = A.take<float>(pl.cb * 3);
        const float* pc = patch + s * mp * 3;

        if (!knn_in) SAPCU_TRY(launch_patch_knn_multi(pc, cb, (int64_t)mp * 3, mp, 3, 3, 3, pl.kk, idx, st));
        for (int l = 0; l < 3; ++l) {
            const int64_t cnt = P * pl.kk[l];
            if (knn_in)
                SAPCU_CHECK_HIP(hipMemcpyAsync(idx[l], knn_in + tab_off[l] + s * mp * pl.kk[l], cnt * 4,
                                               hipMemcpyDeviceToDevice, st));
            if (knn_out)
                SAPCU_CHECK_HIP(hipMemcpyAsync(knn_out + tab_off[l] + s * mp * pl.kk[l], idx[l], cnt * 4,
                                               hipMemcpyDeviceToDevice, st));
        }
        SAPCU_TRY(launch_fn_stem(pc, P, m->p(FN_STEM_W), m->p(FN_STEM_B), m->p(FN_STEM_LIF), m->T, feat0, st));
        SAPCU_TRY(tap_copy(taps, SAPCU_FN_TAP_STEM, s * mp * 64 * 4, feat0, P * 64 * 4, st));

        const float* fin = feat0;
        int ldin = 64;
        for (int l = 0; l < 3; ++l) {
            const int d = 128 << l;
            const int kk = pl.kk[l];
            const int64_t R = P * kk;
            const int sb = FN_BLK0 + l * B_SLOTS;
            const int SP = m->sf16 ? 1 : 0;
            SAPCU_TRY(gemm(m, fin, P, 64, ldin, m->p(sb + B_FC1_W), d, m->p(sb + B_FC1_B), X, d, EPI_LIF, st,
                           m->p(sb + B_SNN1), 4, nullptr, 0, SP << 1));
            SAPCU_TRY(gemm(m, X, P, d, d, m->p(sb + B_QKV_W), 3 * d, m->p(sb + B_QKV_B), QKV, 3 * d, EPI_LIF, st,
                           m->p(sb + B_QKV_LIF), 4, nullptr, 0, SP));
            const float sqrt_hd = (float)sqrt((double)(d / m->heads));
            if (fn_block_fused(m, l, mp)) {
                ChainArgs ca;
                memset(&ca, 0, sizeof(ca));
                ca.P = P; ca.m = mp; ca.qkv = QKV; ca.ldq = 3 * d;
                ca.wd = m->p(sb + B_DELTA_W); ca.bd = m->p(sb + B_DELTA_B); ca.lifd = m->p(sb + B_DELTA_LIF);
                static const int64_t cw_off[3] = {0, (int64_t)3 * 2 * 128 * 128, (int64_t)3 * 2 * (128 * 128 + 256 * 256)};
                const _Float16* cw = (const _Float16*)m->chain_w + cw_off[l];
                ca.w1p = cw; ca.b1 = m->p(sb + B_DELTA2_B); ca.lif1 = m->p(sb + B_DELTA2_LIF);
                ca.w2p = cw + (int64_t)d * d * 2; ca.b2 = m->p(sb + B_GAMMA_B); ca.lif2 = m->p(sb + B_GAMMA_LIF);
                ca.w3p = cw + (int64_t)2 * d * d * 2; ca.b3 = m->p(sb + B_GAMMA2_B);
                ca.inv_sqrt_hd = 1.0f / sqrt_hd;
                ca.res = RES; ca.res_split = SP; ca.T = 4; ca.wide_offsets = m->opt_chain_wide ? 1 : 0;
                SAPCU_TRY(launch_fn_edge_chain(ca, pc, idx[l], d, kk, tab, pdiff, st));
            } else {
                SAPCU_TRY(launch_fn_pe1(pc, idx[l], R, mp, kk, d, m->p(sb + B_DELTA_W), m->p(sb + B_DELTA_B),
                                        m->p(sb + B_DELTA_LIF), 4, B1, SP, st));
                {
                    GemmArgs g;
                    memset(&g, 0, sizeof(g));
                    g.a = B1; g.r = R; g.k = d; g.lda = d; g.w = m->p(sb + B_DELTA2_W); g.n = d;
                    g.bias = m->p(sb + B_DELTA2_B); g.c = B2; g.ldc = d; g.epi = EPI_LIF_ATTN;
                    g.lif = m->p(sb + B_DELTA2_LIF); g.lif_T = 4; g.c2 = B3;
                    g.q = QKV; g.kf = QKV + d; g.ldq = 3 * d; g.tab = tab;
                    g.a_split = SP; g.c2_split = SP;
                    SAPCU_TRY(launch_edge_table(idx[l], R, mp, kk, tab, st));
                    SAPCU_TRY(run_gemm(m, g, st));
                }
                SAPCU_TRY(gemm(m, B3, R, d, d, m->p(sb + B_GAMMA_W), d, m->p(sb + B_GAMMA_B), B1, d, EPI_LIF, st,
                               m->p(sb + B_GAMMA_LIF), 4, nullptr, 0, SP | (SP << 1)));
                {
                    SAPCU_TRY(gemm(m, B1, R, d, d, m->p(sb + B_GAMMA2_W), d, m->p(sb + B_GAMMA2_B), B3, d, EPI_BIAS, st, nullptr, 0,
                                   nullptr, 0, SP));
                    SAPCU_TRY(launch_fn_softmax_agg(B3, B2, QKV + 2 * d, 3 * d, idx[l], P, mp, kk, d, sqrt_hd, RES, SP, st));
                }
            }
            if (m->opt_fn_fold_out) {
                SAPCU_TRY(gemm(m, RES, P, d, d, m->blob + m->fold_w[l], 64, m->blob + m->fold_b[l], cat + 64 * l, 192, EPI_RESID, st,
                               nullptr, 0, fin, ldin, SP));
            } else {
                SAPCU_TRY(gemm(m, RES, P, d, d, m->p(sb + B_OUT_W), d, m->p(sb + B_OUT_B), X, d, EPI_BIAS, st, nullptr, 0, nullptr,
                               0, SP | (SP << 1)));
                SAPCU_TRY(gemm(m, X, P, d, d, m->p(sb + B_FC2_W), 64, m->p(sb + B_FC2_B), cat + 64 * l, 192, EPI_RESID, st,
                               nullptr, 0, fin, ldin, SP));
            }
            if (taps && taps[SAPCU_FN_TAP_BLOCK1 + l]) {
                SAPCU_CHECK_HIP(hipMemcpy2DAsync((char*)taps[SAPCU_FN_TAP_BLOCK1 + l] + s * mp * 64 * 4, 64 * 4,
                                                 cat + 64 * l, 192 * 4, 64 * 4, (size_t)P, hipMemcpyDeviceToDevice, st));
            }
            fin = cat + 64 * l;
            ldin = 192;
        }
        if (m->sf16 && m->opt_fn_maxfuse) {
            GemmArgs g;
            memset(&g, 0, sizeof(g));
            g.a = cat; g.r = P; g.k = 192; g.lda = 192; g.w = m->p(FN_FINAL_W); g.n = m->emb; g.bias = m->p(FN_FINAL_B);
            g.ldc = m->emb; g.epi = EPI_LIF_MAX; g.lif = m->p(FN_FINAL_LIF); g.lif_T = m->T;
            g.max_keys = reinterpret_cast<unsigned*>(B1); g.max_m = mp;
            SAPCU_CHECK_HIP(hipMemsetAsync(g.max_keys, 0, (size_t)cb * m->emb * 4, st));
            SAPCU_TRY(run_gemm(m, g, st));
            SAPCU_TRY(launch_decode_max_keys(g.max_keys, cb * m->emb, pooled, st));
        } else {
            SAPCU_TRY(gemm(m, cat, P, 192, 192, m->p(FN_FINAL_W), m->emb, m->p(FN_FINAL_B), B1, m->emb, EPI_LIF, st,
                           m->p(FN_FINAL_LIF), m->T));
            SAPCU_TRY(launch_rowgroup_max(B1, cb, mp, m->emb, pooled, st));
        }
        SAPCU_TRY(tap_copy(taps, SAPCU_FN_TAP_POOLED, s * m->emb * 4, pooled, cb * m->emb * 4, st));
        SAPCU_TRY(gemm(m, pooled, cb, m->emb, m->emb, m->p(FN_FCOUT_W), 2048, m->p(FN_FCOUT_B), enc, 2048, EPI_BIAS, st));
        SAPCU_TRY(tap_copy(taps, SAPCU_FN_TAP_ENC, s * 2048 * 4, enc, cb * 2048 * 4, st));
        SAPCU_TRY(gemm(m, enc, cb, 2048, 2048, m->p(FN_MLP0_W), 1024, m->p(FN_MLP0_B), h1, 1024, EPI_GELU, st));
        SAPCU_TRY(gemm(m, h1, cb, 1024, 1024, m->p(FN_MLP1_W), 512, m->p(FN_MLP1_B), h2, 512, EPI_GELU, st));
        SAPCU_TRY(gemm(m, h2, cb, 512, 512, m->p(FN_MLP2_W), 256, m->p(FN_MLP2_B), h3, 256, EPI_GELU, st));
        SAPCU_TRY(launch_fn_tail(h3, cb, 256, m->p(FN_HEAD_W), m->p(FN_HEAD_B), m->p(FN_LN_W), m->p(FN_LN_B), logits,
                                 normals + s * 3, st));
        SAPCU_TRY(tap_copy(taps, SAPCU_FN_TAP_LOGITS, s * 3 * 4, logits, cb * 3 * 4, st));
    }
    return SAPCU_OK;
}

struct FdPlan {
    int64_t cb;
    int kmax0, kk;
    bool fused;
    bool x0path;
    bool maxfuse;
    int64_t agg_rows(int mp) const { return maxfuse ? 1 : mp; }
};

static bool fd_encoder_fused(const sapcu_model* m, int mp) {
    return m->sf16 && m->opt_fd_fused && m->fde_w && m->fde_nprm && fd_encoder_ok(mp, m->nscale, m->emb, m->T);
}

static bool fd_x0_path(const sapcu_model* m, int mp) {
    return !fd_encoder_fused(m, mp) && m->sf16 && m->opt_fd_fused && m->opt_fd_x0 && m->opt_fd_maxfuse && m->opt_fd_split && m->fde_w &&
           m->fde_nprm && fd_msc_ok(mp, m->emb, m->T);
}

static FdPlan fd_plan(const sapcu_model* m, int64_t b, int mp) {
    FdPlan pl;
    pl.fused = fd_encoder_fused(m, mp);
    pl.x0path = fd_x0_path(m, mp);
    pl.maxfuse = m->sf16 && m->opt_fd_maxfuse;
    if (pl.fused) {
        const int64_t per_patch_f = ((int64_t)(m->T + 1) * m->emb + 256 + 3 * 128 + 3 * 64 + 192 + 64) * 4;
        pl.cb = chunk_patches(m, b, per_patch_f);
        int kmaxf = 1;
        for (int i = 0; i < m->nscale; ++i) kmaxf = kmaxf > m->ks[i] ? kmaxf : m->ks[i];
        pl.kmax0 = imin(kmaxf, mp);
        pl.kk = imin(m->k, mp);
        return pl;
    }
    int kmax0 = 1;
    for (int i = 0; i < m->nscale; ++i) kmax0 = kmax0 > m->ks[i] ? kmax0 : m->ks[i];
    const int64_t slabs = pl.x0path ? 2 : m->T;
    const int64_t per_patch = (int64_t)mp * ((slabs * 960 + 960 + 1024 + 64 * (m->nscale + 1)) * 4 +
                                            (int64_t)(imin(kmax0, mp) + 3 * imin(m->k, mp)) * 4) +
                              (int64_t)m->T * pl.agg_rows(mp) * m->emb * 4 +
                              ((int64_t)(m->T + 1) * m->emb + 256 + 3 * 128 + 3 * 64 + 192 + 64) * 4;
    pl.cb = chunk_patches(m, b, per_patch);
    int kmax = 1;
    for (int i = 0; i < m->nscale; ++i) kmax = kmax > m->ks[i] ? kmax : m->ks[i];
    pl.kmax0 = imin(kmax, mp);
    pl.kk = imin(m->k, mp);
    return pl;
}

static int64_t fd_ws_bytes(const sapcu_model* m, int64_t b, int mp) {
    const FdPlan pl = fd_plan(m, b, mp);
    const int64_t P = pl.cb * mp;
    int64_t fl = 0;
    auto add = [&](int64_t n, int64_t esz) { fl += ((n * esz) + 255) & ~(int64_t)255; };
    if (!pl.fused) {
        add(P * pl.kmax0, 4); add(3 * P * pl.kk, 4);
        add(P * 64 * m->nscale, 4); add(P * 64, 4);
        add((pl.x0path ? 1 : (int64_t)m->T) * P * 960, 4); add(P * 960, 4); add(P * 1024, 4); add((int64_t)m->T * pl.cb * pl.agg_rows(mp) * m->emb, 4);
        if (pl.x0path) add(P * 960, 4);
    }
    add((int64_t)m->T * pl.cb * m->emb, 4); add(pl.cb * m->emb, 4);
    add(pl.cb * 256, 4);
    for (int i = 0; i < 3; ++i) add(pl.cb * 128, 4);
    for (int i = 0; i < 3; ++i) add(pl.cb * 64, 4);
    add(pl.cb * 192, 4); add(pl.cb * 64, 4);
    return fl + 256;
}

static int fd_forward(const sapcu_model* m, const float* patch, int64_t b, int mp, const int32_t* knn_force,
                      float* dist, void* ws, int64_t ws_bytes, void* const* taps, hipStream_t st) {
    const FdPlan pl = fd_plan(m, b, mp);
    if (ws_bytes < fd_ws_bytes(m, b, mp)) {
        set_error("fd_forward: workspace %lld B < required %lld B", (long long)ws_bytes, (long long)fd_ws_bytes(m, b, mp));
        return SAPCU_ERR_WORKSPACE;
    }
    const int T = m->T, emb = m->emb;
    static const int cin[4] = {0, 64, 128, 256}, cout[4] = {64, 128, 256, 512}, coff[4] = {0, 64, 192, 448};
    for (int64_t s = 0; s < b; s += pl.cb) {
        const int64_t cb = (b - s) < pl.cb ? (b - s) : pl.cb;
        const int64_t P = cb * mp;
        Arena A{(char*)(((uintptr_t)ws + 255) & ~(uintptr_t)255), ws_bytes, 0};
        const int64_t pp = pl.fused ? 0 : 1;
        int32_t* idx0 = A.take<int32_t>(pp * pl.cb * mp * pl.kmax0);
        int32_t* idxb = A.take<int32_t>(pp * 3 * pl.cb * mp * pl.kk);
        float* E0 = A.take<float>(pp * pl.cb * mp * 64 * m->nscale);
        float* FUSED = A.take<float>(pp * pl.cb * mp * 64);
        float* SPK = A.take<float>(pp * (pl.x0path ? 1 : (int64_t)T) * pl.cb * mp * 960);
        float* F0 = A.take<float>(pp * pl.cb * mp * 960);
        float* AB = A.take<float>(pp * pl.cb * mp * 1024);
        float* AGG = A.take<float>(pp * (int64_t)T * pl.cb * pl.agg_rows(mp) * emb);
        float* X0 = A.take<float>(pl.x0path ? pl.cb * mp * 960 : 0);
        float* POOLED = A.take<float>((int64_t)T * pl.cb * emb);
        float* ENC = A.take<float>(pl.cb * emb);
        float* D1 = A.take<float>(pl.cb * 256);
        float* D2a = A.take<float>(pl.cb * 128);
        float* D2b = A.take<float>(pl.cb * 128);
        float* D2c = A.take<float>(pl.cb * 128);
        float* D3a = A.take<float>(pl.cb * 64);
        float* D3b = A.take<float>(pl.cb * 64);
        float* D3c = A.take<float>(pl.cb * 64);
        float* QKV = A.take<float>(pl.cb * 192);
        float* ATT = A.take<float>(pl.cb * 64);
        const float* pc = patch + s * mp * 3;

        if (pl.fused) {
            FdEncArgs ea;
            memset(&ea, 0, sizeof(ea));
            ea.patch = pc; ea.b = cb; ea.b_total = b; ea.s0 = s;
            ea.m = mp; ea.T = T; ea.kk = pl.kk; ea.kmax0 = pl.kmax0; ea.nscale = m->nscale; ea.emb = emb;
            for (int i = 0; i < 4; ++i) ea.ks[i] = i < m->nscale ? imin(m->ks[i], mp) : 0;
            ea.e0_w = m->p(FD_E0_W); ea.e0_b = m->p(FD_E0_B);
            const _Float16* fw = (const _Float16*)m->fde_w;
            ea.fuse_wp = fw + m->fde_off[0]; ea.fuse_b = m->p(FD_FUSE_B);
            for (int l = 0; l < 3; ++l) {
                ea.edge_wp[l] = fw + m->fde_off[1 + l];
                ea.shift[l] = m->p(FD_EDGE1_SHIFT + 3 * l);
            }
            ea.msc_wp = fw + m->fde_off[4]; ea.msc_b = m->p(FD_MSC_B);
            ea.nprm = m->fde_nprm;
            ea.pooled = POOLED;
            ea.knn_force = knn_force;
            ea.tap_knn = taps ? (int32_t*)taps[SAPCU_FD_TAP_KNN] : nullptr;
            ea.tap_fused0 = taps ? (float*)taps[SAPCU_FD_TAP_FUSED0] : nullptr;
            ea.tap_spikes = taps ? (float*)taps[SAPCU_FD_TAP_SPIKES] : nullptr;
            ea.tap_x0 = taps ? (float*)taps[SAPCU_FD_TAP_X0] : nullptr;
            ea.gate = m->gate_dev; ea.ovf = m->ovf_dev;
            SAPCU_TRY(launch_fd_encoder(ea, st));
        } else {
        SAPCU_TRY(launch_patch_knn(pc, cb, mp, 3, 3, pl.kmax0, idx0, st));
        SAPCU_TRY(launch_fd_edge0(pc, idx0, pl.kmax0, P, mp, m->nscale, m->ks_dev, m->p(FD_E0_W), m->p(FD_E0_B), E0, st));
        SAPCU_TRY(gemm(m, E0, P, 64 * m->nscale, 64 * m->nscale, m->p(FD_FUSE_W), 64, m->p(FD_FUSE_B), FUSED, 64,
                       EPI_LRELU, st));
        SAPCU_TRY(tap_copy(taps, SAPCU_FD_TAP_FUSED0, s * mp * 64 * 4, FUSED, P * 64 * 4, st));
        float* const X0T = (taps && taps[SAPCU_FD_TAP_X0]) ? (float*)taps[SAPCU_FD_TAP_X0] + s * mp * 960 : nullptr;
        if (X0T) SAPCU_CHECK_HIP(hipMemcpy2DAsync(X0T, 960 * 4, FUSED, 64 * 4, 64 * 4, (size_t)P, hipMemcpyDeviceToDevice, st));
// ... 168 lines not shown
}

int sapcu_patch_knn(const float* feat, int64_t b, int m, int c, int ld, int k, int32_t* idx_out, void* stream) {
    SAPCU_CHECK_ARG(feat && idx_out && b >= 0 && ld >= c, "patch_knn: bad argument");
    return launch_patch_knn(feat, b, m, c, ld, k, idx_out, (hipStream_t)stream);
}

int sapcu_l2_normalize3(const float* in, float* out, int64_t b, void* stream) {
    SAPCU_CHECK_ARG(in && out && b >= 0, "l2_normalize3: bad argument");
    return launch_l2_normalize3(in, out, b, (hipStream_t)stream);
}

static int split_into_ws(const float* w, int64_t cnt, void* w16_ws, GemmArgs& g, hipStream_t st) {
    char* base = (char*)w16_ws;
    int* ovf = (int*)(base + 4 * cnt);
    SAPCU_CHECK_HIP(hipMemsetAsync(ovf, 0, sizeof(int), st));
    SAPCU_TRY(launch_split_weights(w, cnt, base, base + 2 * cnt, ovf, st));
    g.w16_hi = (const _Float16*)base;
    g.w16_lo = (const _Float16*)(base + 2 * cnt);
    g.ovf = ovf;
    return SAPCU_OK;
}

int sapcu_gemm_f32(const float* a, int64_t r, int k, int lda, const float* w, int n, const float* bias,
                   const float* lif4, int lif_steps, float* c, int ldc, void* w16_ws, int a_split_rows, int c_split_rows,
                   void* stream) {
    SAPCU_CHECK_ARG(a && w && c && r >= 0 && n >= 1, "gemm: bad argument");
    SAPCU_CHECK_ARG(!lif4 || lif_steps >= 1, "gemm: lif_steps must be >= 1");
    SAPCU_CHECK_ARG(!(a_split_rows || c_split_rows) || w16_ws, "gemm: split rows need the split-f16 kernels (w16_ws)");
    SAPCU_CHECK_ARG(r == 0 || (k > 0 && k % 32 == 0 && lda >= k && ldc >= n), "gemm: need k %% 32 == 0, lda >= k and ldc >= n (k=%d lda=%d n=%d ldc=%d)", k, lda, n, ldc);
    SAPCU_CHECK_ARG(r == 0 || ((((uintptr_t)a | (uintptr_t)w | (uintptr_t)w16_ws) & 15) == 0 && lda % (a_split_rows ? 8 : 4) == 0),
                    "gemm: A, W and w16_ws must be 16-byte aligned, lda %% 4 == 0 (%% 8 for split rows) (lda=%d)", lda);
    GemmArgs g;
    memset(&g, 0, sizeof(g));
    g.a = a; g.r = r; g.k = k; g.lda = lda; g.w = w; g.n = n; g.bias = bias; g.c = c; g.ldc = ldc;
    g.epi = lif4 ? EPI_LIF : EPI_BIAS; g.lif = lif4; g.lif_T = lif_steps;
    g.a_split = a_split_rows ? 1 : 0; g.c_split = c_split_rows ? 1 : 0;
    if (w16_ws && (g.a_split || k % 64 == 0)) {
        SAPCU_TRY(split_into_ws(w, (int64_t)n * k, w16_ws, g, (hipStream_t)stream));
        return g.a_split ? launch_gemm_split_rows(g, (hipStream_t)stream, a_split_rows != 2) : launch_gemm_sf16(g, (hipStream_t)stream);
    }
    SAPCU_CHECK_ARG(!g.c_split, "gemm: split-row output needs k %% 64 == 0 on the f32-A path");
    return launch_gemm(g, (hipStream_t)stream);
}

int sapcu_to_split_rows(const float* in, int64_t rows, int k, int ld_in, float* out, int ld_out, void* stream) {
    SAPCU_CHECK_ARG(in && out && rows >= 0 && k >= 1 && ld_in >= k && ld_out >= k, "to_split_rows: bad argument");
    return launch_to_split_rows(in, rows, k, ld_in, out, ld_out, (hipStream_t)stream);
}

int sapcu_posenc_gemm_f32(const float* pe1, int64_t r, int d, const float* w, const float* bias, const float* lif4,
                          int lif_steps, const float* qkv, const int32_t* idx, int kk, int m_pts, float* pe_out,
                          float* attn_in_out, void* edge_table_ws, void* w16_ws, int split_rows, void* stream) {
    SAPCU_CHECK_ARG(pe1 && w && lif4 && qkv && idx && pe_out && attn_in_out && edge_table_ws && r >= 0 && d >= 32 &&
                        lif_steps >= 1 && kk >= 1 && m_pts >= 1,
                    "posenc_gemm: bad argument");
    SAPCU_CHECK_ARG(!split_rows || w16_ws, "posenc_gemm: split rows need the split-f16 kernels (w16_ws)");
    SAPCU_CHECK_ARG(d % 32 == 0, "posenc_gemm: d=%d must be a multiple of 32", d);
    SAPCU_CHECK_ARG((((uintptr_t)pe1 | (uintptr_t)w | (uintptr_t)w16_ws) & 15) == 0 && ((uintptr_t)edge_table_ws & 7) == 0,
                    "posenc_gemm: pe1, w and w16_ws must be 16-byte aligned, edge_table_ws 8-byte aligned");
    GemmArgs g;
    memset(&g, 0, sizeof(g));
    g.a = pe1; g.r = r; g.k = d; g.lda = d; g.w = w; g.n = d; g.bias = bias; g.c = pe_out; g.ldc = d;
    g.epi = EPI_LIF_ATTN; g.lif = lif4; g.lif_T = lif_steps; g.c2 = attn_in_out;
    g.q = qkv; g.kf = qkv + d; g.ldq = 3 * d; g.tab = (const int2*)edge_table_ws;
    SAPCU_TRY(launch_edge_table(idx, r, m_pts, kk, (int2*)edge_table_ws, (hipStream_t)stream));
    if (w16_ws && (split_rows || d % 64 == 0)) {
        SAPCU_TRY(split_into_ws(w, (int64_t)d * d, w16_ws, g, (hipStream_t)stream));
        if (split_rows) {
            g.a_split = 1;
            g.c2_split = 1;
            return launch_gemm_split_rows(g, (hipStream_t)stream, split_rows != 2);
        }
        return launch_gemm_sf16(g, (hipStream_t)stream);
    }
    return launch_gemm(g, (hipStream_t)stream);
}

int64_t sapcu_fn_edge_chain_workspace_bytes(int64_t points, int d, int kk) {
    if (points < 0 || !fn_edge_chain_ok(d, kk)) {
        set_error("fn_edge_chain_workspace_bytes: unsupported shape (d=%d kk=%d)", d, kk);
        return SAPCU_ERR_ARG;
    }
    const int64_t rows = points * kk;
    auto up = [](int64_t b) { return (b + 255) & ~(int64_t)255; };
    return up(rows * 8) + up(rows * 16) + 3 * (up((int64_t)d * d * 4 + 16) + up((int64_t)d * d * 4)) + 256;
}

int sapcu_fn_edge_chain_f32(const float* patch, const int32_t* idx, int64_t points, int m_pts, int d, int kk,
                            const float* qkv, const float* w_delta, const float* b_delta, const float* lif_delta,
                            const float* w1, const float* b1, const float* lif1, const float* w2, const float* b2,
                            const float* lif2, const float* w3, const float* b3, int heads, int lif_steps,
                            float* res_out, void* workspace, int64_t workspace_bytes, void* stream) {
    SAPCU_CHECK_ARG(patch && idx && qkv && w_delta && b_delta && lif_delta && w1 && b1 && lif1 && w2 && b2 && lif2 && w3 && b3 &&
                        res_out && workspace, "fn_edge_chain: null pointer");
    SAPCU_CHECK_ARG(fn_edge_chain_ok(d, kk), "fn_edge_chain: unsupported shape (d=%d kk=%d)", d, kk);
    SAPCU_CHECK_ARG(points >= 0 && m_pts >= kk && heads >= 1 && d % heads == 0 && lif_steps >= 1, "fn_edge_chain: bad sizes");
    const int64_t need = sapcu_fn_edge_chain_workspace_bytes(points, d, kk);
    if (workspace_bytes < need) {
        set_error("fn_edge_chain: workspace %lld B < required %lld B", (long long)workspace_bytes, (long long)need);
        return SAPCU_ERR_WORKSPACE;
    }
    hipStream_t st = (hipStream_t)stream;
    Arena A{(char*)(((uintptr_t)workspace + 255) & ~(uintptr_t)255), workspace_bytes, 0};
    int2* tab = A.take<int2>(points * kk);
    float4* pd = A.take<float4>(points * kk);
    const float* ws[3] = {w1, w2, w3};
    const _Float16* packed[3];
    for (int q = 0; q < 3; ++q) {
        char* split = A.take<char>((int64_t)d * d * 4 + 16);
        _Float16* pk = A.take<_Float16>((int64_t)d * d * 2);
        GemmArgs g;
        memset(&g, 0, sizeof(g));
        SAPCU_TRY(split_into_ws(ws[q], (int64_t)d * d, split, g, st));
        SAPCU_TRY(launch_pack_chain_weights(g.w16_hi, g.w16_lo, d, pk, st));
        packed[q] = pk;
    }
    ChainArgs ca;
    memset(&ca, 0, sizeof(ca));
    ca.P = points; ca.m = m_pts; ca.qkv = qkv; ca.ldq = 3 * d;
    ca.wd = w_delta; ca.bd = b_delta; ca.lifd = lif_delta;
    ca.w1p = packed[0]; ca.b1 = b1; ca.lif1 = lif1;
    ca.w2p = packed[1]; ca.b2 = b2; ca.lif2 = lif2;
    ca.w3p = packed[2]; ca.b3 = b3;
    ca.inv_sqrt_hd = 1.0f / (float)sqrt((double)(d / heads));
    ca.res = res_out; ca.res_split = 0; ca.T = lif_steps;
    return launch_fn_edge_chain(ca, patch, idx, d, kk, tab, pd, st);
}

int sapcu_model_create(int kind, const int32_t* hp, int n_hp, const float* blob, int64_t blob_floats,
                       const int64_t* dir_host, int n_dir, sapcu_model_t* out) {
    SAPCU_CHECK_ARG(hp && blob && dir_host && out && blob_floats > 0, "model_create: null pointer");
    sapcu_model* m = new (std::nothrow) sapcu_model();
    SAPCU_CHECK_ARG(m != nullptr, "model_create: out of host memory");
    m->kind = kind;
    m->ks_dev = nullptr;
    m->gate_dev = nullptr;
    m->blob = nullptr;
    m->w16_hi = nullptr;
    m->w16_lo = nullptr;
    m->chain_w = nullptr;
    m->ovf_dev = nullptr;
    m->fde_w = nullptr;
    m->fde_nprm = nullptr;
    const char* ge = getenv("SAPCU_GEMM");
    m->sf16 = !(ge && strcmp(ge, "f32") == 0);
    m->opt_bt = !env_off("SAPCU_BT");
    m->opt_chain = !env_off("SAPCU_CHAIN");
    {
        const char* v = getenv("SAPCU_CHAIN");
        m->opt_chain_wide = v && strcmp(v, "wide") == 0;
    }
    m->opt_fn_maxfuse = !env_off("SAPCU_FN_MAXFUSE");
    m->opt_fn_fold_out = !env_off("SAPCU_FN_FOLD_OUT");
    for (int l = 0; l < 3; ++l) m->fold_w[l] = m->fold_b[l] = 0;
    m->opt_fd_maxfuse = !env_off("SAPCU_FD_MAXFUSE");
    m->opt_fd_split = !env_off("SAPCU_FD_SPLIT");
    m->opt_fd_fused = !env_off("SAPCU_FD_FUSED");
    m->opt_fd_x0 = !env_off("SAPCU_FD_X0");
    const char* ce = getenv("SAPCU_CHUNK");
    m->chunk = ce ? atoll(ce) : 0;
    if (m->chunk < 0) m->chunk = 0;
    const char* be = getenv("SAPCU_WS_BUDGET_MB");
    m->ws_budget = (be ? atoll(be) : 20480) * (int64_t)(1 << 20);
    if (m->ws_budget < (int64_t)(64 << 20)) m->ws_budget = (int64_t)(64 << 20);
    int rc = SAPCU_OK;
    if (kind == SAPCU_KIND_FN) {
        if (n_hp != 6 || n_dir != FN_SLOTS) {
            set_error("model_create(fn): need 6 hparams and %d slots (got %d, %d)", (int)FN_SLOTS, n_hp, n_dir);
            rc = SAPCU_ERR_ARG;
        } else {
            m->kv[0] = hp[0]; m->kv[1] = hp[1]; m->kv[2] = hp[2];
            m->emb = hp[3]; m->T = hp[4]; m->heads = hp[5];
            if (m->kv[0] < 1 || m->kv[1] < 1 || m->kv[2] < 1 || m->emb < 32 || m->emb % 32 || m->T < 1 || m->heads < 1 ||
                128 % m->heads) {
                set_error("model_create(fn): unsupported hyper-parameters");
                rc = SAPCU_ERR_ARG;
            }
        }
    } else if (kind == SAPCU_KIND_FD) {
        if (n_hp < 6 || n_dir != FD_SLOTS || hp[4] < 1 || hp[4] > 8 || n_hp != 5 + hp[4]) {
            set_error("model_create(fd): need [k,emb,T,heads,S,ks...] and %d slots", (int)FD_SLOTS);
            rc = SAPCU_ERR_ARG;
        } else {
            m->k = hp[0]; m->emb = hp[1]; m->T = hp[2]; m->heads = hp[3]; m->nscale = hp[4];
            for (int i = 0; i < m->nscale; ++i) m->ks[i] = hp[5 + i];
            if (m->k < 1 || m->emb < 32 || m->emb % 32 || m->T < 1 || m->T > 64 || m->heads < 1) {
                set_error("model_create(fd): unsupported hyper-parameters");
                rc = SAPCU_ERR_ARG;
            }
        }
    } else {
        set_error("model_create: unknown kind %d", kind);
        rc = SAPCU_ERR_ARG;
    }
    if (rc == SAPCU_OK) {
        m->dir.assign(dir_host, dir_host + n_dir);
        for (int i = 0; i < n_dir; ++i)
            if (m->dir[i] < 0 || m->dir[i] >= blob_floats || (m->dir[i] & 3)) {
                set_error("model_create: slot %d offset %lld out of range / unaligned", i, (long long)m->dir[i]);
                rc = SAPCU_ERR_ARG;
                break;
            }
    }
    auto hip_ok = [&](hipError_t e, const char* what) {
        if (e != hipSuccess && rc == SAPCU_OK) {
            set_error("model_create: %s failed: %s", what, hipGetErrorString(e));
            rc = SAPCU_ERR_HIP;
        }
    };
    if (rc == SAPCU_OK) {
        int64_t total = blob_floats;
        if (kind == SAPCU_KIND_FN && m->opt_fn_fold_out) {
            total = (total + 63) & ~(int64_t)63;
            for (int l = 0; l < 3; ++l) {
                m->fold_w[l] = total;
                total += (int64_t)64 * (128 << l);
                m->fold_b[l] = total;
                total += 64;
            }
        }
        m->blob_floats = total;
        hip_ok(hipMalloc((void**)&m->blob, (size_t)total * 4), "hipMalloc(blob)");
        if (rc == SAPCU_OK) hip_ok(hipMemcpy(m->blob, blob, (size_t)blob_floats * 4, hipMemcpyDeviceToDevice), "copy blob");
        if (rc == SAPCU_OK && total > blob_floats)
            hip_ok(hipMemset(m->blob + blob_floats, 0, (size_t)(total - blob_floats) * 4), "memset folded parameters");
        for (int l = 0; l < 3 && rc == SAPCU_OK && total > blob_floats; ++l) {
            const int d = 128 << l, sb = FN_BLK0 + l * B_SLOTS;
            const int64_t need[4] = {(int64_t)d * d, d, (int64_t)64 * d, 64};
            static const int slot[4] = {B_OUT_W, B_OUT_B, B_FC2_W, B_FC2_B};
            std::vector<float> h[4], wf((size_t)64 * d), bf(64);
            for (int q = 0; q < 4 && rc == SAPCU_OK; ++q) {
                if (m->dir[sb + slot[q]] + need[q] > blob_floats) {
                    set_error("model_create(fn): slot %d runs past the end of the blob", sb + slot[q]);
                    rc = SAPCU_ERR_ARG;
                    break;
                }
                h[q].resize((size_t)need[q]);
                hip_ok(hipMemcpy(h[q].data(), m->p(sb + slot[q]), (size_t)need[q] * 4, hipMemcpyDeviceToHost), "read out_proj / fc2");
            }
            if (rc != SAPCU_OK) break;
            fold_affine_f64(h[0].data(), h[1].data(), h[2].data(), h[3].data(), d, 64, wf.data(), bf.data());
            hip_ok(hipMemcpy(m->blob + m->fold_w[l], wf.data(), wf.size() * 4, hipMemcpyHostToDevice), "copy folded weights");
            if (rc == SAPCU_OK) hip_ok(hipMemcpy(m->blob + m->fold_b[l], bf.data(), bf.size() * 4, hipMemcpyHostToDevice), "copy folded bias");
        }
        if (rc == SAPCU_OK) hip_ok(hipMalloc((void**)&m->ovf_dev, 2 * sizeof(int)), "hipMalloc(ovf)");
        if (rc == SAPCU_OK) hip_ok(hipMemset(m->ovf_dev, 0, 2 * sizeof(int)), "memset ovf");
        if (rc == SAPCU_OK && m->sf16) {
            hip_ok(hipMalloc(&m->w16_hi, (size_t)total * 2), "hipMalloc(w16_hi)");
            if (rc == SAPCU_OK) hip_ok(hipMalloc(&m->w16_lo, (size_t)total * 2), "hipMalloc(w16_lo)");
            if (rc == SAPCU_OK) {
                int wovf = 0;
                if (launch_split_weights(m->blob, total, m->w16_hi, m->w16_lo, m->ovf_dev + 1, nullptr) != SAPCU_OK)
                    rc = SAPCU_ERR_HIP;
                if (rc == SAPCU_OK) hip_ok(hipMemcpy(&wovf, m->ovf_dev + 1, sizeof(int), hipMemcpyDeviceToHost), "read ovf");
                if (rc == SAPCU_OK && wovf != 0) m->sf16 = false;
            }
            if (rc == SAPCU_OK && m->sf16 && kind == SAPCU_KIND_FN) {
                const int64_t halves = (int64_t)3 * 2 * (128 * 128 + 256 * 256 + 512 * 512);
                hip_ok(hipMalloc(&m->chain_w, (size_t)halves * 2), "hipMalloc(chain_w)");
                int64_t off = 0;
                for (int l = 0; l < 3 && rc == SAPCU_OK; ++l) {
                    const int d = 128 << l;
                    static const int slots[3] = {B_DELTA2_W, B_GAMMA_W, B_GAMMA2_W};
                    for (int q = 0; q < 3 && rc == SAPCU_OK; ++q) {
                        const int64_t wo = m->dir[FN_BLK0 + l * B_SLOTS + slots[q]];
                        if (launch_pack_chain_weights((const _Float16*)m->w16_hi + wo, (const _Float16*)m->w16_lo + wo, d,
                                                      (_Float16*)m->chain_w + off, nullptr) != SAPCU_OK)
                            rc = SAPCU_ERR_HIP;
                        off += (int64_t)d * d * 2;
                    }
                }
                if (rc == SAPCU_OK) hip_ok(hipDeviceSynchronize(), "pack chain weights");
            }
        }
        if (rc == SAPCU_OK && kind == SAPCU_KIND_FD) {
            hip_ok(hipMalloc((void**)&m->ks_dev, 8 * sizeof(int32_t)), "hipMalloc(ks)");
            if (rc == SAPCU_OK) hip_ok(hipMemcpy(m->ks_dev, m->ks, 8 * sizeof(int32_t), hipMemcpyHostToDevice), "copy ks");
            if (rc == SAPCU_OK) hip_ok(hipMalloc((void**)&m->gate_dev, sizeof(int)), "hipMalloc(gate)");
            if (rc == SAPCU_OK) hip_ok(hipMemset(m->gate_dev, 0, sizeof(int)), "memset gate");
            if (rc == SAPCU_OK && m->sf16 && m->nscale <= 4 && m->emb >= 96) {
                const int mats[5][3] = {{FD_FUSE_W, 64, 64 * m->nscale}, {FD_EDGE1_W, 256, 64}, {FD_EDGE2_W, 512, 128},
                                        {FD_EDGE3_W, 1024, 256}, {FD_MSC_W, m->emb, 960}};
                int64_t halves = 0;
                for (int i = 0; i < 5; ++i) {
                    m->fde_off[i] = halves;
                    halves += (int64_t)2 * mats[i][1] * mats[i][2];
                }
                hip_ok(hipMalloc(&m->fde_w, (size_t)halves * 2), "hipMalloc(fde_w)");
                if (rc == SAPCU_OK) hip_ok(hipMalloc((void**)&m->fde_nprm, 960 * 8 * sizeof(float)), "hipMalloc(fde_nprm)");
                for (int i = 0; i < 5 && rc == SAPCU_OK; ++i) {
                    const int64_t wo = m->dir[mats[i][0]];
                    if (launch_pack_frag_weights((const _Float16*)m->w16_hi + wo, (const _Float16*)m->w16_lo + wo, mats[i][1], mats[i][2],
                                                 (_Float16*)m->fde_w + m->fde_off[i], nullptr) != SAPCU_OK)
                        rc = SAPCU_ERR_HIP;
                }
                static const int nslot[4] = {FD_SNN0, FD_SNN1, FD_SNN2, FD_SNN3}, nch[4] = {64, 128, 256, 512}, noff[4] = {0, 64, 192, 448};
                for (int i = 0; i < 4 && rc == SAPCU_OK; ++i)
                    if (launch_pack_fd_neuron(m->p(nslot[i]), nch[i], i < 2 ? 1 : 0, noff[i], m->fde_nprm, nullptr) != SAPCU_OK) rc = SAPCU_ERR_HIP;
                if (rc == SAPCU_OK) hip_ok(hipDeviceSynchronize(), "pack fd encoder operands");
            }
        }
    }
    if (rc != SAPCU_OK) {
        if (m->w16_hi) (void)hipFree(m->w16_hi);
        if (m->w16_lo) (void)hipFree(m->w16_lo);
        if (m->chain_w) (void)hipFree(m->chain_w);
        if (m->ovf_dev) (void)hipFree(m->ovf_dev);
        if (m->blob) (void)hipFree(m->blob);
        if (m->ks_dev) (void)hipFree(m->ks_dev);
        if (m->gate_dev) (void)hipFree(m->gate_dev);
        if (m->fde_w) (void)hipFree(m->fde_w);
        if (m->fde_nprm) (void)hipFree(m->fde_nprm);
        delete m;
        return rc;
    }
    *out = m;
    return SAPCU_OK;
}

int sapcu_internal_fold_affine_host(const float* w_out, const float* b_out, const float* w_fc2, const float* b_fc2, int d, int n,
                                    float* w_fold_out, float* b_fold_out) {
    SAPCU_CHECK_ARG(w_out && b_out && w_fc2 && b_fc2 && w_fold_out && b_fold_out && d >= 1 && n >= 1, "fold_affine: bad argument");
    fold_affine_f64(w_out, b_out, w_fc2, b_fc2, d, n, w_fold_out, b_fold_out);
    return SAPCU_OK;
}

int sapcu_model_destroy(sapcu_model_t m) {
    if (!m) return SAPCU_OK;
    if (m->w16_hi) (void)hipFree(m->w16_hi);
    if (m->w16_lo) (void)hipFree(m->w16_lo);
    if (m->chain_w) (void)hipFree(m->chain_w);
    if (m->ovf_dev) (void)hipFree(m->ovf_dev);
    if (m->blob) (void)hipFree(m->blob);
    if (m->ks_dev) (void)hipFree(m->ks_dev);
    if (m->gate_dev) (void)hipFree(m->gate_dev);
    if (m->fde_w) (void)hipFree(m->fde_w);
    if (m->fde_nprm) (void)hipFree(m->fde_nprm);
    delete m;
    return SAPCU_OK;
}

int64_t sapcu_workspace_bytes(sapcu_model_t m, int64_t b, int m_pts) {
    if (!m || b < 0 || m_pts < 1 || m_pts > 128) {
        set_error("workspace_bytes: bad argument");
        return SAPCU_ERR_ARG;
    }
    return m->kind == SAPCU_KIND_FN ? fn_ws_bytes(m, b, m_pts) : fd_ws_bytes(m, b, m_pts);
}

int sapcu_model_gate_violations(sapcu_model_t m, int* count_host) {
    SAPCU_CHECK_ARG(m && count_host, "gate_violations: null pointer");
    *count_host = 0;
    if (m->gate_dev) SAPCU_CHECK_HIP(hipMemcpy(count_host, m->gate_dev, sizeof(int), hipMemcpyDeviceToHost));
    return SAPCU_OK;
}

int sapcu_model_gemm_mode(sapcu_model_t m, int* split_f16_host, int* range_overflows_host) {
    SAPCU_CHECK_ARG(m && split_f16_host && range_overflows_host, "gemm_mode: null pointer");
    *split_f16_host = m->sf16 ? 1 : 0;
    *range_overflows_host = 0;
    if (m->ovf_dev) SAPCU_CHECK_HIP(hipMemcpy(range_overflows_host, m->ovf_dev, sizeof(int), hipMemcpyDeviceToHost));
    return SAPCU_OK;
}

int sapcu_model_fused_blocks(sapcu_model_t m, int m_pts, int* mask_host) {
    SAPCU_CHECK_ARG(m && mask_host && m_pts >= 1 && m_pts <= 128, "fused_blocks: bad argument");
    int mask = 0;
    if (m->kind == SAPCU_KIND_FN) {
        for (int l = 0; l < 3; ++l)
            if (fn_block_fused(m, l, m_pts)) mask |= 1 << l;
    } else {
        if (fd_encoder_fused(m, m_pts)) mask = 1;
        else if (fd_x0_path(m, m_pts)) mask = 2;
    }
    *mask_host = mask;
    return SAPCU_OK;
}

int sapcu_fn_forward(sapcu_model_t m, const float* patch, int64_t b, int m_pts, const int32_t* knn_in, int32_t* knn_out,
                     float* normals_out, void* workspace, int64_t ws_bytes, void* const* taps_host, void* stream) {
    SAPCU_CHECK_ARG(m && m->kind == SAPCU_KIND_FN, "fn_forward: not an fn model handle");
    SAPCU_CHECK_ARG(patch && normals_out && workspace, "fn_forward: null pointer");
    SAPCU_CHECK_ARG(b >= 0 && m_pts >= 1 && m_pts <= 128, "fn_forward: need 1 <= m_pts <= 128 (got %d)", m_pts);
    return fn_forward(m, patch, b, m_pts, knn_in, knn_out, normals_out, workspace, ws_bytes, taps_host,
                      (hipStream_t)stream);
}

int sapcu_fd_forward(sapcu_model_t m, const float* patch, int64_t b, int m_pts, const int32_t* knn_force, float* dist_out,
                     void* workspace, int64_t ws_bytes, void* const* taps_host, void* stream) {
    SAPCU_CHECK_ARG(m && m->kind == SAPCU_KIND_FD, "fd_forward: not an fd model handle");
    SAPCU_CHECK_ARG(patch && dist_out && workspace, "fd_forward: null pointer");
    SAPCU_CHECK_ARG(b >= 0 && m_pts >= 1 && m_pts <= 128, "fd_forward: need 1 <= m_pts <= 128 (got %d)", m_pts);
    return fd_forward(m, patch, b, m_pts, knn_force, dist_out, workspace, ws_bytes, taps_host, (hipStream_t)stream);
}

}
```

c-users-sayakdutta-self-supervised-arbitrary-scale-point-cloud-upsampling-via-snn_amd/csrc/ops.h:

```cpp
#pragma once
#include "common.h"

namespace sapcu {

int launch_patch_knn_strided(const float* feat, int64_t b, int64_t pstride, int m, int c, int ld, int k,
                             int32_t* idx, hipStream_t st);
int launch_patch_knn_multi(const float* feat, int64_t b, int64_t pstride, int m, int c, int ld, int ntab,
                           const int* ks, int32_t* const* idx, hipStream_t st);
int launch_patch_knn(const float* feat, int64_t b, int m, int c, int ld, int k, int32_t* idx, hipStream_t st);
int launch_neuron_selfloop(const float* x, int64_t rows, int ch, int T, const float* md, const float* ta,
                           const float* rd, const float* tb, const float* dT, const float* rh, float* so, float* mo,
                           float* to, float* ro, hipStream_t st);
int launch_neuron_drive(const float* x, int64_t rows, int ch, int T, const float* md, const float* ta, const float* rd, const float* tb,
                        const float* dT, const float* rh, int pairv, float* so, float* mo, float* to, float* ro, int* gate, hipStream_t st);
int launch_fn_stem(const float* patch, int64_t rows, const float* w, const float* bias, const float* lif, int T,
                   float* out, hipStream_t st);
int launch_fn_pe1(const float* patch, const int32_t* idx, int64_t rows, int m, int kk, int d, const float* w,
                  const float* bias, const float* lif, int T, float* out, int split, hipStream_t st);
struct ChainArgs {
    int64_t P;
    int m;
    const int2* tab;
    const float4* pd;
    const float* qkv;
    int ldq;
    const float* wd;
    const float* bd;
    const float* lifd;
    const _Float16* w1p;
    const float* b1;
    const float* lif1;
    const _Float16* w2p;
    const float* b2;
    const float* lif2;
    const _Float16* w3p;
    const float* b3;
    float inv_sqrt_hd;
    float* res;
    int res_split;
    int T;
    int wide_offsets;
};
bool fn_edge_chain_ok(int d, int kk);
int launch_fn_edge_chain(ChainArgs a, const float* patch, const int32_t* idx, int d, int kk, int2* tab_ws, float4* pd_ws,
                         hipStream_t st);
int launch_pack_chain_weights(const void* w16_hi, const void* w16_lo, int d, void* out, hipStream_t st);
int launch_edge_table(const int32_t* idx, int64_t rows, int m, int kk, int2* tab, hipStream_t st);
int launch_fn_softmax_agg(const float* a, const float* pe, const float* v, int ldv, const int32_t* idx, int64_t pts,
                          int m, int kk, int d, float sqrt_hd, float* res, int split, hipStream_t st);
int launch_decode_max_keys(const unsigned* keys, int64_t count, float* out, hipStream_t st);
int launch_rowgroup_max(const float* in, int64_t groups, int m, int c, float* out, hipStream_t st);
int launch_fn_tail(const float* h, int64_t b, int kdim, const float* w, const float* bias, const float* lnw,
                   const float* lnb, float* logits, float* normals, hipStream_t st);
int launch_to_split_rows(const float* in, int64_t rows, int k, int ld_in, float* out, int ld_out, hipStream_t st);
int launch_l2_normalize3(const float* in, float* out, int64_t b, hipStream_t st);
int launch_fd_edge0(const float* patch, const int32_t* idx, int kmax, int64_t pts, int m, int nscale,
                    const int32_t* ks_dev, const float* w, const float* bias, float* out, hipStream_t st);
int launch_fd_neuron(bool eif, int mode, const float* in, int ldi, const int32_t* idx, int kk, int m,
                     const float* shift, int64_t pts, int C, const float* prm, int T, float* spk, int ldo, int coff,
                     float* pre_out, int* gate_violations, hipStream_t st, float* spk_split = nullptr,
                     float* x0_out = nullptr);
typedef _Float16 fe_half8 __attribute__((ext_vector_type(8)));
struct FdEncArgs {
    const float* patch;
    int64_t b;
    int64_t b_total, s0;
    int m, T, kk, kmax0, nscale, emb;
    int ks[4];
    const float* e0_w;
    const float* e0_b;
    const _Float16* fuse_wp;
    const float* fuse_b;
    const _Float16* edge_wp[3];
    const float* shift[3];
    const _Float16* msc_wp;
    const float* msc_b;
    const float* nprm;
    float* pooled;
    const int32_t* knn_force;
    int32_t* tap_knn;
    float* tap_fused0;
    float* tap_spikes;
    float* tap_x0;
    int* gate;
    int* ovf;
};
struct FdMscArgs {
    const float* x0;
    int64_t b;
    int64_t b_total, s0;
    int m, T, emb;
    const _Float16* msc_wp;
    const float* msc_b;
    const float* nprm;
    float* pooled;
    float* tap_spikes;
    int* gate;
};
bool fd_msc_ok(int m, int emb, int T);
int launch_fd_msc(const FdMscArgs& a, hipStream_t st);
bool fd_encoder_ok(int m, int nscale, int emb, int T);
int launch_fd_encoder(const FdEncArgs& a, hipStream_t st);
int launch_pack_frag_weights(const void* w16_hi, const void* w16_lo, int n, int k, void* out, hipStream_t st);
int launch_pack_fd_neuron(const float* raw, int C, int eif, int coff, float* out, hipStream_t st);
int launch_fd_pre(const float* in, int ldi, const int32_t* idx, int kk, int m, const float* shift, int64_t pts, int C, float* out,
                  int ldo, int coff, hipStream_t st);
int launch_fd_temporal(const float* pooled, int T, int64_t b, int emb, const float* tw, const float* lif, float* out,
                       hipStream_t st);
int launch_fd_tail(const float* x, const float* qkv, int64_t b, int heads, const float* wo_t, const float* bo,
                   const float* lnw, const float* lnb, const float* wh_t, const float* bh, const float* wd,
                   const float* bd, float* attn_out, float* dist, hipStream_t st);

}
```

c-users-sayakdutta-self-supervised-arbitrary-scale-point-cloud-upsampling-via-snn_amd/csrc/patch_ops.hip:

```cpp
#include "common.h"
#include "ops.h"
#include "gemm_epi.h"

namespace sapcu {

constexpr int PK_CH = 32;

struct KnnOut {
    int32_t* idx[3];
    int k[3];
    int n;
};

constexpr int PK_LD = 36;

template <int NT>
__global__ __launch_bounds__(NT) void patch_knn_kernel(const float* __restrict__ feat, int64_t pstride, int m,
                                                       int c, int ld, const KnnOut out) {
    extern __shared__ float sm[];
    unsigned* K = reinterpret_cast<unsigned*>(sm);
    float* xx = sm + m * (m + 1);
    float* F = xx + m;
    const int tid = threadIdx.x;
    const int lane = tid & 63, wave = __builtin_amdgcn_readfirstlane(tid >> 6);
// ... 134 lines not shown
    for (int t = 0; t < 3; ++t) {
        out.idx[t] = t < ntab ? idx[t] : nullptr;
        out.k[t] = t < ntab ? ks[t] : 0;
        if (t < ntab) SAPCU_CHECK_ARG(ks[t] >= 1 && ks[t] <= m && idx[t], "patch_knn: need 1<=k<=m (k=%d m=%d)", ks[t], m);
    }
    const int nb = (m + 15) / 16;
    const size_t lds = (size_t)(m * (m + 1) + m + 16 * nb * PK_LD) * sizeof(float);
#define SAPCU_PK(NT)                                                                                                  \
    do {                                                                                                              \
        static DeviceOnce once;                                                                                       \
        if (lds > 65536) SAPCU_SET_MAX_LDS(once, (&patch_knn_kernel<NT>), 98304);                                      \
        hipLaunchKernelGGL((patch_knn_kernel<NT>), dim3((unsigned)b), dim3(NT), lds, st, feat, pstride, m, c, ld, out); \
    } while (0)
    if (m <= 64) SAPCU_PK(256);
    else SAPCU_PK(512);
#undef SAPCU_PK
    SAPCU_CHECK_LAUNCH();
    return SAPCU_OK;
}

int launch_patch_knn_strided(const float* feat, int64_t b, int64_t pstride, int m, int c, int ld, int k,
                             int32_t* idx, hipStream_t st) {
    return launch_patch_knn_multi(feat, b, pstride, m, c, ld, 1, &k, &idx, st);
}

int launch_patch_knn(const float* feat, int64_t b, int m, int c, int ld, int k, int32_t* idx, hipStream_t st) {
    return launch_patch_knn_strided(feat, b, (int64_t)m * ld, m, c, ld, k, idx, st);
}

template <bool EIF, bool PAIRV>
__global__ __launch_bounds__(256) void neuron_drive_kernel(const float* __restrict__ x, int64_t rows, int ch, int T, const float* md,
                                                           const float* ta, const float* rd, const float* tb, const float* dT,
                                                           const float* rh, float* __restrict__ so, float* mo, float* to, float* ro,
                                                           int* __restrict__ gate) {
    const int64_t t = (int64_t)blockIdx.x * blockDim.x + threadIdx.x;
    const int64_t npair = PAIRV ? rows * ((ch + 1) / 2) : ((rows + 1) / 2) * ch;
    if (t >= npair) return;
    int64_t ea, eb;
    int ca, cb;
    if (PAIRV) {
        const int hc = (ch + 1) / 2;
        const int64_t r = t / hc;
        ca = 2 * (int)(t % hc);
        cb = ca + 1 < ch ? ca + 1 : ca;
        ea = r * ch + ca;
        eb = r * ch + cb;
    } else {
        ca = cb = (int)(t % ch);
        const int64_t r = 2 * (t / ch), r1 = r + 1 < rows ? r + 1 : r;
        ea = r * ch + ca;
        eb = r1 * ch + cb;
    }
    auto prm = [&](int c) {
        NeuronP p;
        p.decay = clampf(md[c], 0.1f, 0.99f);
        p.adapt = clampf(ta[c], 0.001f, 0.1f);
        p.rdecay = clampf(rd[c], 0.1f, 0.95f);
        p.theta0 = tb[c];
        p.dT = EIF ? clampf(dT[c], 0.1f, 5.0f) : 0.f;
        p.rh = EIF ? clampf(rh[c], 0.1f, 2.0f) : 0.f;
        return p;
    };
    const f32x2 xin = f32x2{x[ea], x[eb]}, z = f32x2{0.f, 0.f};
    int open = 0;
    f32x2 m2, th2, r2;
    auto run = [&](auto& n) {
        for (int step = 0; step < T; ++step) {
            if (step > 0 && n.gate_open()) ++open;
            const f32x2 sp = n.step(step == 0 ? xin : z, step == 0);
            if (so) {
                so[(int64_t)step * rows * ch + ea] = sp.x;
                so[(int64_t)step * rows * ch + eb] = sp.y;
            }
        }
#ifdef SAPCU_LIF_EXACT_ORDER
        m2 = f32x2{n.sx.m, n.sy.m}; th2 = f32x2{n.sx.th, n.sy.th}; r2 = f32x2{n.sx.r, n.sy.r};
#else
        m2 = n.s.m; th2 = n.s.th; r2 = n.s.r;
#endif
    };
    if (PAIRV) {
        NeuronStep2V<EIF> n(prm(ca), prm(cb));
        run(n);
    } else {
        NeuronStep2<EIF> n(prm(ca));
        run(n);
    }
    if (mo) { mo[ea] = m2.x; mo[eb] = m2.y; }
    if (to) { to[ea] = th2.x; to[eb] = th2.y; }
    if (ro) { ro[ea] = r2.x; ro[eb] = r2.y; }
    if (open && gate) atomicAdd(gate, open);
}

int launch_neuron_drive(const float* x, int64_t rows, int ch, int T, const float* md, const float* ta, const float* rd, const float* tb,
                        const float* dT, const float* rh, int pairv, float* so, float* mo, float* to, float* ro, int* gate, hipStream_t st) {
    const int64_t npair = pairv ? rows * ((ch + 1) / 2) : ((rows + 1) / 2) * ch;
    if (npair == 0) return SAPCU_OK;
    const dim3 grid((unsigned)((npair + 255) / 256)), blk(256);
#define SAPCU_ND(E, V) hipLaunchKernelGGL((neuron_drive_kernel<E, V>), grid, blk, 0, st, x, rows, ch, T, md, ta, rd, tb, dT, rh, so, mo, to, ro, gate)
    if (dT && pairv) SAPCU_ND(true, true);
    else if (dT) SAPCU_ND(true, false);
    else if (pairv) SAPCU_ND(false, true);
    else SAPCU_ND(false, false);
#undef SAPCU_ND
    SAPCU_CHECK_LAUNCH();
    return SAPCU_OK;
}

template <bool EIF>
__global__ __launch_bounds__(256) void neuron_selfloop_kernel(const float* __restrict__ x, int64_t total, int ch,
                                                              int T, const float* md, const float* ta,
                                                              const float* rd, const float* tb, const float* dT,
                                                              const float* rh, float* so, float* mo, float* to,
                                                              float* ro) {
    const int64_t t = (int64_t)blockIdx.x * blockDim.x + threadIdx.x;
    if (t >= total) return;
    const int c = (int)(t % ch);
    NeuronP p;
    p.decay = clampf(md[c], 0.1f, 0.99f);
    p.adapt = clampf(ta[c], 0.001f, 0.1f);
    p.rdecay = clampf(rd[c], 0.1f, 0.95f);
    p.theta0 = tb[c];
    p.dT = EIF ? clampf(dT[c], 0.1f, 5.0f) : 0.f;
    p.rh = EIF ? clampf(rh[c], 0.1f, 2.0f) : 0.f;
    NeuronS s = neuron_init(p);
    float v = x[t];
    for (int i = 0; i < T; ++i) v = neuron_step<EIF>(v, s, p);
    if (!EIF) v = lif_selfloop(x[t], p, T);
    if (so) so[t] = v;
    if (mo) mo[t] = s.m;
    if (to) to[t] = s.th;
    if (ro) ro[t] = s.r;
}

int launch_neuron_selfloop(const float* x, int64_t rows, int ch, int T, const float* md, const float* ta,
                           const float* rd, const float* tb, const float* dT, const float* rh, float* so, float* mo,
                           float* to, float* ro, hipStream_t st) {
    const int64_t total = rows * ch;
    if (total == 0) return SAPCU_OK;
    const unsigned grid = (unsigned)((total + 255) / 256);
    if (dT)
        hipLaunchKernelGGL(neuron_selfloop_kernel<true>, dim3(grid), dim3(256), 0, st, x, total, ch, T, md, ta, rd, tb,
                           dT, rh, so, mo, to, ro);
    else
        hipLaunchKernelGGL(neuron_selfloop_kernel<false>, dim3(grid), dim3(256), 0, st, x, total, ch, T, md, ta, rd,
                           tb, dT, rh, so, mo, to, ro);
    SAPCU_CHECK_LAUNCH();
    return SAPCU_OK;
}

__global__ __launch_bounds__(256) void fn_stem_kernel(const float* __restrict__ patch, int64_t rows,
                                                      const float* __restrict__ w ,
                                                      const float* __restrict__ bias, const float* __restrict__ lif,
                                                      int T, float* __restrict__ out) {
    const int64_t t = (int64_t)blockIdx.x * blockDim.x + threadIdx.x;
    if (t >= rows * 64) return;
    const int c = (int)(t & 63);
    const int64_t r = t >> 6;
    const float x = patch[r * 3], y = patch[r * 3 + 1], z = patch[r * 3 + 2];
    float a = __fmul_rn(w[c * 3], x);
    a = __fmaf_rn(w[c * 3 + 1], y, a);
    a = __fmaf_rn(w[c * 3 + 2], z, a);
    a = __fadd_rn(a, bias[c]);
    out[t] = lif_selfloop(a, load_lif(lif, 64, c), T);
}

int launch_fn_stem(const float* patch, int64_t rows, const float* w, const float* bias, const float* lif, int T,
                   float* out, hipStream_t st) {
    if (rows == 0) return SAPCU_OK;
    hipLaunchKernelGGL(fn_stem_kernel, dim3((unsigned)((rows * 64 + 255) / 256)), dim3(256), 0, st, patch, rows, w,
                       bias, lif, T, out);
    SAPCU_CHECK_LAUNCH();
    return SAPCU_OK;
}

constexpr int PE_ROWS = 32;

__global__ __launch_bounds__(256) void fn_pe1_kernel(const float* __restrict__ patch, const int32_t* __restrict__ idx,
                                                     int64_t rows, int m, int kk, int d,
                                                     const float* __restrict__ w ,
                                                     const float* __restrict__ bias, const float* __restrict__ lif,
                                                     int T, float* __restrict__ out, int split) {
    __shared__ float pd[PE_ROWS][3];
    const int64_t row0 = (int64_t)blockIdx.x * PE_ROWS;
    const int c = blockIdx.y * blockDim.x + threadIdx.x;
    if (threadIdx.x < PE_ROWS) {
        const int64_t r = row0 + threadIdx.x;
        float dx = 0.f, dy = 0.f, dz = 0.f;
        if (r < rows) {
            const int64_t pt = r / kk;
            const int64_t patch_i = pt / m;
            const float* pi = patch + pt * 3;
            const float* pj = patch + (patch_i * m + idx[r]) * 3;
            dx = __fsub_rn(pi[0], pj[0]);
            dy = __fsub_rn(pi[1], pj[1]);
            dz = __fsub_rn(pi[2], pj[2]);
        }
        pd[threadIdx.x][0] = dx;
        pd[threadIdx.x][1] = dy;
        pd[threadIdx.x][2] = dz;
    }
    __syncthreads();
    if (c >= d) return;
    const float w0 = w[c * 3], w1 = w[c * 3 + 1], w2 = w[c * 3 + 2], bb = bias[c];
    const NeuronP np = load_lif(lif, d, c);
    const int nrow = (int)((rows - row0) < PE_ROWS ? (rows - row0) : PE_ROWS);
    for (int r4 = 0; r4 < nrow; r4 += 4) {
        float v[4];
#pragma unroll
        for (int u = 0; u < 4; ++u) {
            const int rr = r4 + u < PE_ROWS ? r4 + u : PE_ROWS - 1;
            float a = __fmul_rn(w0, pd[rr][0]);
            a = __fmaf_rn(w1, pd[rr][1], a);
            a = __fmaf_rn(w2, pd[rr][2], a);
            v[u] = __fadd_rn(a, bb);
        }
        lif_selfloop_n<4>(v, np, T);
#pragma unroll
        for (int u = 0; u < 4; ++u)
            if (r4 + u < nrow) {
                if (split) store_split(out, row0 + r4 + u, d, c, v[u]);
                else out[(row0 + r4 + u) * d + c] = v[u];
            }
    }
}

__global__ __launch_bounds__(256) void fn_pe1_vec4_kernel(const float* __restrict__ patch, const int32_t* __restrict__ idx,
                                                          int64_t rows, int m, int kk, int d,
                                                          const float* __restrict__ w ,
                                                          const float* __restrict__ bias, const float* __restrict__ lif,
                                                          int T, float* __restrict__ out, int split) {
    __shared__ float pd[PE_ROWS][3];
    const int tpr = d >> 2;
    const int rpp = 256 / tpr;
    const int rsub = threadIdx.x / tpr;
    const int c = (threadIdx.x - rsub * tpr) * 4;
    float wx[4], wy[4], wz[4];
#pragma unroll
    for (int u = 0; u < 4; ++u) {
        wx[u] = w[(c + u) * 3];
        wy[u] = w[(c + u) * 3 + 1];
        wz[u] = w[(c + u) * 3 + 2];
    }
    const float4 bb = ld4(bias + c);
    const float4 pdc = ld4(lif + c), pad = ld4(lif + d + c), prd = ld4(lif + 2 * (int64_t)d + c), pth = ld4(lif + 3 * (int64_t)d + c);
    NeuronP2 np[2];
    np[0].decay = f32x2{clampf(pdc.x, 0.1f, 0.99f), clampf(pdc.y, 0.1f, 0.99f)};
    np[1].decay = f32x2{clampf(pdc.z, 0.1f, 0.99f), clampf(pdc.w, 0.1f, 0.99f)};
    np[0].adapt = f32x2{clampf(pad.x, 0.001f, 0.1f), clampf(pad.y, 0.001f, 0.1f)};
    np[1].adapt = f32x2{clampf(pad.z, 0.001f, 0.1f), clampf(pad.w, 0.001f, 0.1f)};
    np[0].rdecay = f32x2{clampf(prd.x, 0.1f, 0.95f), clampf(prd.y, 0.1f, 0.95f)};
    np[1].rdecay = f32x2{clampf(prd.z, 0.1f, 0.95f), clampf(prd.w, 0.1f, 0.95f)};
    np[0].theta0 = f32x2{pth.x, pth.y};
    np[1].theta0 = f32x2{pth.z, pth.w};
    const NeuronP2 np4[4] = {np[0], np[1], np[0], np[1]};
    const float bs[4] = {bb.x, bb.y, bb.z, bb.w};
    const int64_t nstrips = (rows + PE_ROWS - 1) / PE_ROWS;
    for (int64_t strip = blockIdx.x; strip < nstrips; strip += gridDim.x) {
        const int64_t row0 = strip * PE_ROWS;
        __syncthreads();
        if (threadIdx.x < PE_ROWS) {
            const int64_t r = row0 + threadIdx.x;
            float dx = 0.f, dy = 0.f, dz = 0.f;
            if (r < rows) {
                const int64_t pt = r / kk;
                const int64_t patch_i = pt / m;
                const float* pi = patch + pt * 3;
                const float* pj = patch + (patch_i * m + idx[r]) * 3;
                dx = __fsub_rn(pi[0], pj[0]);
                dy = __fsub_rn(pi[1], pj[1]);
                dz = __fsub_rn(pi[2], pj[2]);
            }
            pd[threadIdx.x][0] = dx;
            pd[threadIdx.x][1] = dy;
            pd[threadIdx.x][2] = dz;
        }
        __syncthreads();
        const int nrow = (int)((rows - row0) < PE_ROWS ? (rows - row0) : PE_ROWS);
        for (int r = rsub; r < nrow; r += 2 * rpp) {
            const int rb = r + rpp < PE_ROWS ? r + rpp : r;
            float va[4], vb[4];
#pragma unroll
            for (int u = 0; u < 4; ++u) {
                float a = __fmul_rn(wx[u], pd[r][0]);
                a = __fmaf_rn(wy[u], pd[r][1], a);
                a = __fmaf_rn(wz[u], pd[r][2], a);
                va[u] = __fadd_rn(a, bs[u]);
                float b2 = __fmul_rn(wx[u], pd[rb][0]);
                b2 = __fmaf_rn(wy[u], pd[rb][1], b2);
                b2 = __fmaf_rn(wz[u], pd[rb][2], b2);
                vb[u] = __fadd_rn(b2, bs[u]);
            }
            f32x2 pv[4] = {f32x2{va[0], va[1]}, f32x2{va[2], va[3]}, f32x2{vb[0], vb[1]}, f32x2{vb[2], vb[3]}};
            lif_selfloop_pairs<4>(pv, np4, T);
            const float oa[4] = {pv[0].x, pv[0].y, pv[1].x, pv[1].y}, ob[4] = {pv[2].x, pv[2].y, pv[3].x, pv[3].y};
            if (split) store_split4<true>(out, row0 + r, d, c, d, oa);
            else store_f32x4<true>(out, row0 + r, d, c, d, oa);
            if (rb != r && rb < nrow) {
                if (split) store_split4<true>(out, row0 + rb, d, c, d, ob);
                else store_f32x4<true>(out, row0 + rb, d, c, d, ob);
            }
        }
    }
}

int launch_fn_pe1(const float* patch, const int32_t* idx, int64_t rows, int m, int kk, int d, const float* w,
                  const float* bias, const float* lif, int T, float* out, int split, hipStream_t st) {
    if (rows == 0) return SAPCU_OK;
    const int64_t strips = (rows + PE_ROWS - 1) / PE_ROWS;
    SAPCU_CHECK_ARG(strips < 0x7fffffffLL, "pe1: too many rows");
    const int tpr = d / 4;
    const bool al16 = (((uintptr_t)bias | (uintptr_t)lif | (uintptr_t)out) & 15) == 0;
    if (d % 4 == 0 && tpr >= 1 && tpr <= 256 && (tpr & (tpr - 1)) == 0 && al16) {
        const int64_t grid = strips < 256 * 40 ? strips : 256 * 40;
        hipLaunchKernelGGL(fn_pe1_vec4_kernel, dim3((unsigned)grid), dim3(256), 0, st, patch, idx, rows, m, kk, d, w, bias, lif,
                           T, out, split);
        SAPCU_CHECK_LAUNCH();
        return SAPCU_OK;
    }
    const int bx = d < 256 ? ((d + 63) / 64) * 64 : 256;
    hipLaunchKernelGGL(fn_pe1_kernel, dim3((unsigned)strips, (unsigned)((d + bx - 1) / bx)), dim3(bx), 0, st, patch, idx,
                       rows, m, kk, d, w, bias, lif, T, out, split);
    SAPCU_CHECK_LAUNCH();
    return SAPCU_OK;
// ... 649 lines not shown
```

Baseline: 125,000 query-points/s.

## Emit split-row copies of point features so FN point GEMMs use big-tile kernel

```diff
diff --git a/c-users-sayakdutta-self-supervised-arbitrary-scale-point-cloud-upsampling-via-snn_amd/_lib.py b/c-users-sayakdutta-self-supervised-arbitrary-scale-point-cloud-upsampling-via-snn_amd/_lib.py
--- a/c-users-sayakdutta-self-supervised-arbitrary-scale-point-cloud-upsampling-via-snn_amd/_lib.py
+++ b/c-users-sayakdutta-self-supervised-arbitrary-scale-point-cloud-upsampling-via-snn_amd/_lib.py
@@ -88,6 +88,9 @@
 SEEDS_EXPORTS = tuple(_SEEDS_SIGNATURES)
 
 _INTERNAL_SIGNATURES = {
+    "sapcu_internal_fn_point_route": (c_int, [c_void_p, c_int64, c_int, c_void_p]),
+    "sapcu_internal_gemm_lif_max": (c_int, [c_void_p, c_int64, c_int, c_int, c_void_p, c_int, c_void_p, c_void_p, c_int, c_int, c_void_p,
+                                            c_void_p, c_void_p, c_int, c_void_p]),
     "sapcu_internal_fold_affine_host": (c_int, [c_void_p, c_void_p, c_void_p, c_void_p, c_int, c_int, c_void_p, c_void_p]),
 }
 _lib = None
diff --git a/c-users-sayakdutta-self-supervised-arbitrary-scale-point-cloud-upsampling-via-snn_amd/csrc/gemm_epi.h b/c-users-sayakdutta-self-supervised-arbitrary-scale-point-cloud-upsampling-via-snn_amd/csrc/gemm_epi.h
--- a/c-users-sayakdutta-self-supervised-arbitrary-scale-point-cloud-upsampling-via-snn_amd/csrc/gemm_epi.h
+++ b/c-users-sayakdutta-self-supervised-arbitrary-scale-point-cloud-upsampling-via-snn_amd/csrc/gemm_epi.h
@@ -56,7 +56,9 @@
     }
 #pragma unroll
     for (int u = 0; u < W; ++u) v[u] = __fadd_rn(acc[u], bias);
+#ifndef SAPCU_TIMING_NO_NEURON
     if (EPI == EPI_LIF || EPI == EPI_LIF_ATTN || EPI == EPI_LIF_MAX) lif_selfloop_n<W>(v, np, g.lif_T);
+#endif
 #pragma unroll
     for (int u = 0; u < W; ++u) {
         if (EPI == EPI_GELU) v[u] = gelu_erf(v[u]);
@@ -200,6 +202,17 @@
     }
 }
 
+template <bool VEC>
+__device__ __forceinline__ void count_f16_range4(const GemmArgs& g, const float (&v)[4], int col) {
+    if (!g.ovf) return;
+    float big = 0.f;
+#pragma unroll
+    for (int u = 0; u < 4; ++u)
+        if (VEC || col + u < g.n) big = fmaxf(big, fabsf(v[u]));
+    const bool nan = (VEC || col < g.n) && !(v[0] == v[0] && v[1] == v[1] && v[2] == v[2] && v[3] == v[3]);
+    if (!(big < 65504.0f) || nan) atomicAdd(g.ovf, 1);
+}
+
 template <int EPI, bool VEC>
 __device__ __forceinline__ void epilogue_row4_store(const GemmArgs& g, const float (&v)[4], int64_t row, int col,
                                                     const float4 q, const float4 kf) {
@@ -213,20 +226,17 @@
     }
     if (g.c_split) {
         store_split4<VEC>(g.c, row, g.ldc, col, g.n, v);
-        if (EPI != EPI_LIF && EPI != EPI_LIF_ATTN && g.ovf) {
-            float big = 0.f;
-#pragma unroll
-            for (int u = 0; u < 4; ++u)
-                if (VEC || col + u < g.n) big = fmaxf(big, fabsf(v[u]));
-            const bool nan = (VEC || col < g.n) && !(v[0] == v[0] && v[1] == v[1] && v[2] == v[2] && v[3] == v[3]);
-            if (!(big < 65504.0f) || nan) atomicAdd(g.ovf, 1);
-        }
+        if (EPI != EPI_LIF && EPI != EPI_LIF_ATTN) count_f16_range4<VEC>(g, v, col);
     } else {
         store_f32x4<VEC>(g.c, row, g.ldc, col, g.n, v);
     }
     if (EPI == EPI_LIF_ATTN) {
         if (g.c2_split) store_split4<VEC>(g.c2, row, g.ldc, col, g.n, ai);
         else store_f32x4<VEC>(g.c2, row, g.ldc, col, g.n, ai);
+    }
+    if (EPI == EPI_RESID && g.c2) {
+        store_split4<VEC>(g.c2, row, g.ldc, col, g.n, v);
+        count_f16_range4<VEC>(g, v, col);
     }
 }
 
diff --git a/c-users-sayakdutta-self-supervised-arbitrary-scale-point-cloud-upsampling-via-snn_amd/csrc/gemm_f32.hip b/c-users-sayakdutta-self-supervised-arbitrary-scale-point-cloud-upsampling-via-snn_amd/csrc/gemm_f32.hip
--- a/c-users-sayakdutta-self-supervised-arbitrary-scale-point-cloud-upsampling-via-snn_amd/csrc/gemm_f32.hip
+++ b/c-users-sayakdutta-self-supervised-arbitrary-scale-point-cloud-upsampling-via-snn_amd/csrc/gemm_f32.hip
@@ -233,6 +233,7 @@
     SAPCU_CHECK_ARG(g.k > 0 && g.k % BK == 0, "gemm: k=%d must be a positive multiple of %d", g.k, BK);
     SAPCU_CHECK_ARG(g.lda % 4 == 0 && ((uintptr_t)g.a & 15) == 0 && ((uintptr_t)g.w & 15) == 0,
                     "gemm: A/W must be 16-byte aligned with lda %% 4 == 0 (lda=%d)", g.lda);
+    SAPCU_CHECK_ARG(!(g.epi == EPI_RESID && g.c2), "gemm: a split-row copy of C (c2 under EPI_RESID) exists on the ring kernel only");
     switch (g.epi) {
         case EPI_BIAS: return launch_t<EPI_BIAS>(g, st);
         case EPI_LIF: return launch_t<EPI_LIF>(g, st);
diff --git a/c-users-sayakdutta-self-supervised-arbitrary-scale-point-cloud-upsampling-via-snn_amd/csrc/gemm_sf16.hip b/c-users-sayakdutta-self-supervised-arbitrary-scale-point-cloud-upsampling-via-snn_amd/csrc/gemm_sf16.hip
--- a/c-users-sayakdutta-self-supervised-arbitrary-scale-point-cloud-upsampling-via-snn_amd/csrc/gemm_sf16.hip
+++ b/c-users-sayakdutta-self-supervised-arbitrary-scale-point-cloud-upsampling-via-snn_amd/csrc/gemm_sf16.hip
@@ -310,6 +310,7 @@
     SAPCU_CHECK_ARG(g.lda % 4 == 0 && ((uintptr_t)g.a & 15) == 0 && g.w16_hi && g.w16_lo &&
                         ((uintptr_t)g.w16_hi & 15) == 0 && ((uintptr_t)g.w16_lo & 15) == 0,
                     "gemm_sf16: operands must be 16-byte aligned (lda=%d)", g.lda);
+    SAPCU_CHECK_ARG(!(g.epi == EPI_RESID && g.c2), "gemm_sf16: a split-row copy of C (c2 under EPI_RESID) exists on the ring kernel only");
     switch (g.epi) {
         case EPI_BIAS: return launch_t16<EPI_BIAS>(g, st);
         case EPI_LIF: return launch_t16<EPI_LIF>(g, st);
diff --git a/c-users-sayakdutta-self-supervised-arbitrary-scale-point-cloud-upsampling-via-snn_amd/csrc/gemm_sf16_bt.hip b/c-users-sayakdutta-self-supervised-arbitrary-scale-point-cloud-upsampling-via-snn_amd/csrc/gemm_sf16_bt.hip
--- a/c-users-sayakdutta-self-supervised-arbitrary-scale-point-cloud-upsampling-via-snn_amd/csrc/gemm_sf16_bt.hip
+++ b/c-users-sayakdutta-self-supervised-arbitrary-scale-point-cloud-upsampling-via-snn_amd/csrc/gemm_sf16_bt.hip
@@ -300,7 +300,7 @@
             const int col = col0 + j * 16 + c16;
             pbias[j] = 0.f;
             if (g.bias) pbias[j] = bt_load_f32(g.bias + col);
-            if (EPI == EPI_LIF || EPI == EPI_LIF_ATTN) {
+            if (EPI == EPI_LIF || EPI == EPI_LIF_ATTN || EPI == EPI_LIF_MAX) {
 #pragma unroll
                 for (int q = 0; q < 4; ++q) praw[j][q] = bt_load_f32(g.lif + (int64_t)q * g.n + col);
             }
@@ -312,7 +312,7 @@
 #pragma unroll
         for (int j = 0; j < CS; ++j) {
             pnp[j] = NeuronP{0.f, 0.f, 0.f, 0.f, 0.f, 0.f};
-            if (EPI == EPI_LIF || EPI == EPI_LIF_ATTN) {
+            if (EPI == EPI_LIF || EPI == EPI_LIF_ATTN || EPI == EPI_LIF_MAX) {
                 pnp[j].decay = clampf(praw[j][0], 0.1f, 0.99f);
                 pnp[j].adapt = clampf(praw[j][1], 0.001f, 0.1f);
                 pnp[j].rdecay = clampf(praw[j][2], 0.1f, 0.95f);
@@ -345,6 +345,64 @@
                 }
                 if (cur >= 0) atomicMax(g.max_keys + cur * g.n + col, float_max_key(best));
             }
+        } else if (EPI == EPI_LIF_MAX) {
+            const bool fast16 = (g.max_m & 15) == 0 && (g.r & 15) == 0;
+            int64_t cur = -1, boundary = 0;
+            float best[CS];
+#pragma unroll
+            for (int j = 0; j < CS; ++j) best[j] = 0.f;
+            auto flush = [&]() {
+                if (cur < 0 || (fast16 && g4 != 0)) return;
+#pragma unroll
+                for (int j = 0; j < CS; ++j) atomicMax(g.max_keys + cur * g.n + (col0 + j * 16 + c16), float_max_key(best[j]));
+            };
+#pragma unroll
+            for (int rs = 0; rs < 8; ++rs) {
+                const int64_t row = row0 + rs * 16 + 4 * g4;
+                float v[CS][4];
+#pragma unroll
+                for (int j = 0; j < CS; ++j) {
+#pragma unroll
+                    for (int u = 0; u < 4; ++u) v[j][u] = __fadd_rn(__fmul_rn(acc[rs][j][u], 0.0625f), pbias[j]);
+                    lif_selfloop_n<4>(v[j], pnp[j], g.lif_T);
+                }
+                if (fast16) {
+                    const int64_t blk = row0 + rs * 16;
+                    if (blk < g.r) {
+                        const bool fresh = blk >= boundary;
+                        if (fresh) {
+                            flush();
+                            cur = blk / g.max_m;
+                            boundary = (cur + 1) * g.max_m;
+                        }
+#pragma unroll
+                        for (int j = 0; j < CS; ++j) {
+                            float mx = fmaxf(fmaxf(v[j][0], v[j][1]), fmaxf(v[j][2], v[j][3]));
+                            mx = fmaxf(mx, __shfl_xor(mx, 16));
+                            mx = fmaxf(mx, __shfl_xor(mx, 32));
+                            best[j] = fresh ? mx : fmaxf(best[j], mx);
+                        }
+                    }
+                } else {
+#pragma unroll
+                    for (int u = 0; u < 4; ++u) {
+                        const int64_t rr = row + u;
+                        if (rr >= g.r) continue;
+                        if (rr >= boundary) {
+                            flush();
+                            cur = rr / g.max_m;
+                            boundary = (cur + 1) * g.max_m;
+#pragma unroll
+                            for (int j = 0; j < CS; ++j) best[j] = v[j][u];
+                        } else {
+#pragma unroll
+                            for (int j = 0; j < CS; ++j) best[j] = fmaxf(best[j], v[j][u]);
+                        }
+                    }
+                }
+                __builtin_amdgcn_sched_barrier(0);
+            }
+            flush();
         } else if (interior && EPI == EPI_LIF_ATTN && !g.c_split && g.c2_split) {
             bt_epilogue_fast<EPI, CS, false, true>(g, acc, row0, col0, c16, g4, pbias, pnp);
         } else if (interior && EPI == EPI_LIF && g.c_split) {
@@ -405,19 +463,20 @@
     if (g.r < 4 * TBM) return false;
     auto al16 = [](const void* p) { return ((uintptr_t)p & 15) == 0; };
     if (g.ldc % 4 || !al16(g.c) || (g.bias && !al16(g.bias))) return false;
-    if ((g.epi == EPI_LIF || g.epi == EPI_LIF_ATTN) && !al16(g.lif)) return false;
+    if ((g.epi == EPI_LIF || g.epi == EPI_LIF_ATTN || g.epi == EPI_LIF_MAX) && !al16(g.lif)) return false;
     if (g.epi == EPI_LIF_ATTN && (g.ldq % 4 || !al16(g.q) || !al16(g.kf) || !al16(g.c2))) return false;
-    if (g.epi == EPI_LRELU_MAX) return g.max_keys != nullptr && g.max_m >= 1;
+    if (g.epi == EPI_LRELU_MAX || g.epi == EPI_LIF_MAX) return g.max_keys != nullptr && g.max_m >= 1;
     return g.epi == EPI_BIAS || g.epi == EPI_LIF || g.epi == EPI_LIF_ATTN;
 }
 
 int launch_gemm_sf16_bt(const GemmArgs& g, hipStream_t st) {
     if (g.r == 0 || g.n == 0) return SAPCU_OK;
     SAPCU_CHECK_ARG(gemm_sf16_bt_ok(g), "gemm_bt: unsupported shape or epilogue");
-    if (g.epi == EPI_LIF || g.epi == EPI_LIF_ATTN) SAPCU_CHECK_ARG(g.lif, "gemm_bt: missing neuron parameters");
+    if (g.epi == EPI_LIF || g.epi == EPI_LIF_ATTN || g.epi == EPI_LIF_MAX) SAPCU_CHECK_ARG(g.lif, "gemm_bt: missing neuron parameters");
     if (g.epi == EPI_LIF_ATTN) SAPCU_CHECK_ARG(g.ldq > 0 && g.tab && g.q && g.kf && g.c2, "gemm_bt: bad attn operands");
     const bool wide = g.n % 256 == 0;
     switch (g.epi) {
+        case EPI_LIF_MAX: return launch_bt_t<EPI_LIF_MAX, 128>(g, st);
         case EPI_LRELU_MAX: return wide ? launch_bt_t<EPI_LRELU_MAX, 256>(g, st) : launch_bt_t<EPI_LRELU_MAX, 128>(g, st);
         case EPI_BIAS: return wide ? launch_bt_t<EPI_BIAS, 256>(g, st) : launch_bt_t<EPI_BIAS, 128>(g, st);
         case EPI_LIF: return wide ? launch_bt_t<EPI_LIF, 256>(g, st) : launch_bt_t<EPI_LIF, 128>(g, st);
diff --git a/c-users-sayakdutta-self-supervised-arbitrary-scale-point-cloud-upsampling-via-snn_amd/csrc/gemm_sf16_ring.hip b/c-users-sayakdutta-self-supervised-arbitrary-scale-point-cloud-upsampling-via-snn_amd/csrc/gemm_sf16_ring.hip
--- a/c-users-sayakdutta-self-supervised-arbitrary-scale-point-cloud-upsampling-via-snn_amd/csrc/gemm_sf16_ring.hip
+++ b/c-users-sayakdutta-self-supervised-arbitrary-scale-point-cloud-upsampling-via-snn_amd/csrc/gemm_sf16_ring.hip
@@ -341,7 +341,7 @@
     auto al16 = [](const void* p) { return ((uintptr_t)p & 15) == 0; };
     bool ok = g.n % 4 == 0 && g.ldc % 4 == 0 && al16(g.c) && (!g.bias || al16(g.bias));
     if (g.epi == EPI_LIF || g.epi == EPI_LIF_ATTN) ok = ok && al16(g.lif);
-    if (g.epi == EPI_RESID || g.epi == EPI_RESID_GELU) ok = ok && g.ldr % 4 == 0 && al16(g.resid);
+    if (g.epi == EPI_RESID || g.epi == EPI_RESID_GELU) ok = ok && g.ldr % 4 == 0 && al16(g.resid) && al16(g.c2);
     if (g.epi == EPI_LIF_ATTN) ok = ok && g.ldq % 4 == 0 && al16(g.q) && al16(g.kf) && al16(g.c2);
     return ok;
 }
diff --git a/c-users-sayakdutta-self-supervised-arbitrary-scale-point-cloud-upsampling-via-snn_amd/csrc/model.hip b/c-users-sayakdutta-self-supervised-arbitrary-scale-point-cloud-upsampling-via-snn_amd/csrc/model.hip
--- a/c-users-sayakdutta-self-supervised-arbitrary-scale-point-cloud-upsampling-via-snn_amd/csrc/model.hip
+++ b/c-users-sayakdutta-self-supervised-arbitrary-scale-point-cloud-upsampling-via-snn_amd/csrc/model.hip
@@ -79,6 +79,7 @@
     bool opt_chain;
     bool opt_chain_wide;
     bool opt_fn_maxfuse;
+    bool opt_fn_ptsplit;
     bool opt_fn_fold_out;
     bool opt_fd_maxfuse;
     bool opt_fd_split;
@@ -157,14 +158,23 @@
     return launch_gemm(g, st);
 }
 
+static bool split_lif_max_on_big_tile(const sapcu_model* m, GemmArgs g) {
+    if (!m->sf16 || !(g.w >= m->blob && g.w < m->blob + m->blob_floats)) return false;
+    const int64_t off = g.w - m->blob;
+    g.w16_hi = (const _Float16*)m->w16_hi + off;
+    g.w16_lo = (const _Float16*)m->w16_lo + off;
+    return split_rows_gemm_on_big_tile(g, m->opt_bt);
+}
+
 static int gemm(const sapcu_model* m, const float* a, int64_t r, int k, int lda, const float* w, int n,
                 const float* bias, float* c, int ldc, int epi, hipStream_t st, const float* lif = nullptr,
-                int lifT = 0, const float* resid = nullptr, int ldr = 0, int fmt = 0) {
+                int lifT = 0, const float* resid = nullptr, int ldr = 0, int fmt = 0, float* c_copy_split = nullptr) {
     GemmArgs g;
     memset(&g, 0, sizeof(g));
     g.a = a; g.r = r; g.k = k; g.lda = lda; g.w = w; g.n = n; g.bias = bias; g.c = c; g.ldc = ldc;
     g.epi = epi; g.lif = lif; g.lif_T = lifT; g.resid = resid; g.ldr = ldr;
     g.a_split = fmt & 1; g.c_split = (fmt >> 1) & 1;
+    g.c2 = c_copy_split;
     return run_gemm(m, g, st);
 }
 
@@ -190,6 +200,8 @@
 static bool fn_block_fused(const sapcu_model* m, int l, int mp) {
     return m->sf16 && m->chain_w && m->opt_chain && fn_edge_chain_ok(128 << l, imin(m->kv[l], mp));
 }
+
+static bool fn_point_split(const sapcu_model* m) { return m->sf16 && m->opt_fn_ptsplit; }
 
 static void fn_edge_floats_per_patch(const sapcu_model* m, int mp, int64_t& first, int64_t& others) {
     first = (int64_t)mp * m->emb;
@@ -212,7 +224,8 @@
         idxs += (int64_t)mp * kk * 4;
         kmx = kmx > kk ? kmx : kk;
     }
-    return (e1 + 2 * e23) * 4 + idxs + (int64_t)mp * kmx * 24 + (int64_t)mp * (64 + 192 + 512 + 1536 + 512) * 4 +
+    return (e1 + 2 * e23) * 4 + idxs + (int64_t)mp * kmx * 24 +
+           (int64_t)mp * (64 + 192 + 512 + 1536 + 512 + (fn_point_split(m) ? 64 + 192 : 0)) * 4 +
            ((int64_t)m->emb + 2048 + 1024 + 512 + 256 + 3) * 4;
 }
 
@@ -245,6 +258,7 @@
     for (int l = 0; l < 3; ++l) add(P * pl.kk[l], 4);
     { int kmx = 1; for (int l = 0; l < 3; ++l) kmx = kmx > pl.kk[l] ? kmx : pl.kk[l]; add(P * kmx, 8); add(P * kmx, 16); }
     add(P * 64, 4); add(P * 192, 4); add(P * 512, 4); add(P * 1536, 4); add(P * 512, 4);
+    if (fn_point_split(m)) { add(P * 64, 4); add(P * 192, 4); }
     add(pl.edge_floats, 4); add(pl.edge_floats23, 4); add(pl.edge_floats23, 4);
     add(pl.cb * m->emb, 4); add(pl.cb * 2048, 4); add(pl.cb * 1024, 4); add(pl.cb * 512, 4); add(pl.cb * 256, 4);
     add(pl.cb * 3, 4);
@@ -279,6 +293,9 @@
         float* X = A.take<float>(pl.cb * mp * 512);
         float* QKV = A.take<float>(pl.cb * mp * 1536);
         float* RES = A.take<float>(pl.cb * mp * 512);
+        const bool psplit = fn_point_split(m);
+        float* feat0s = psplit ? A.take<float>(pl.cb * mp * 64) : nullptr;
+        float* cats = psplit ? A.take<float>(pl.cb * mp * 192) : nullptr;
         float* B1 = A.take<float>(pl.edge_floats);
         float* B2 = A.take<float>(pl.edge_floats23);
         float* B3 = A.take<float>(pl.edge_floats23);
@@ -300,10 +317,11 @@
                 SAPCU_CHECK_HIP(hipMemcpyAsync(knn_out + tab_off[l] + s * mp * pl.kk[l], idx[l], cnt * 4,
                                                hipMemcpyDeviceToDevice, st));
         }
-        SAPCU_TRY(launch_fn_stem(pc, P, m->p(FN_STEM_W), m->p(FN_STEM_B), m->p(FN_STEM_LIF), m->T, feat0, st));
+        SAPCU_TRY(launch_fn_stem(pc, P, m->p(FN_STEM_W), m->p(FN_STEM_B), m->p(FN_STEM_LIF), m->T, feat0, feat0s, st));
         SAPCU_TRY(tap_copy(taps, SAPCU_FN_TAP_STEM, s * mp * 64 * 4, feat0, P * 64 * 4, st));
 
         const float* fin = feat0;
+        const float* fins = feat0s;
         int ldin = 64;
         for (int l = 0; l < 3; ++l) {
             const int d = 128 << l;
@@ -311,8 +329,8 @@
             const int64_t R = P * kk;
             const int sb = FN_BLK0 + l * B_SLOTS;
             const int SP = m->sf16 ? 1 : 0;
-            SAPCU_TRY(gemm(m, fin, P, 64, ldin, m->p(sb + B_FC1_W), d, m->p(sb + B_FC1_B), X, d, EPI_LIF, st,
-                           m->p(sb + B_SNN1), 4, nullptr, 0, SP << 1));
+            SAPCU_TRY(gemm(m, psplit ? fins : fin, P, 64, ldin, m->p(sb + B_FC1_W), d, m->p(sb + B_FC1_B), X, d, EPI_LIF, st,
+                           m->p(sb + B_SNN1), 4, nullptr, 0, (psplit ? 1 : 0) | (SP << 1)));
             SAPCU_TRY(gemm(m, X, P, d, d, m->p(sb + B_QKV_W), 3 * d, m->p(sb + B_QKV_B), QKV, 3 * d, EPI_LIF, st,
                            m->p(sb + B_QKV_LIF), 4, nullptr, 0, SP));
             const float sqrt_hd = (float)sqrt((double)(d / m->heads));
@@ -353,18 +371,19 @@
             }
             if (m->opt_fn_fold_out) {
                 SAPCU_TRY(gemm(m, RES, P, d, d, m->blob + m->fold_w[l], 64, m->blob + m->fold_b[l], cat + 64 * l, 192, EPI_RESID, st,
-                               nullptr, 0, fin, ldin, SP));
+                               nullptr, 0, fin, ldin, SP, psplit ? cats + 64 * l : nullptr));
             } else {
                 SAPCU_TRY(gemm(m, RES, P, d, d, m->p(sb + B_OUT_W), d, m->p(sb + B_OUT_B), X, d, EPI_BIAS, st, nullptr, 0, nullptr,
                                0, SP | (SP << 1)));
                 SAPCU_TRY(gemm(m, X, P, d, d, m->p(sb + B_FC2_W), 64, m->p(sb + B_FC2_B), cat + 64 * l, 192, EPI_RESID, st,
-                               nullptr, 0, fin, ldin, SP));
+                               nullptr, 0, fin, ldin, SP, psplit ? cats + 64 * l : nullptr));
             }
             if (taps && taps[SAPCU_FN_TAP_BLOCK1 + l]) {
                 SAPCU_CHECK_HIP(hipMemcpy2DAsync((char*)taps[SAPCU_FN_TAP_BLOCK1 + l] + s * mp * 64 * 4, 64 * 4,
                                                  cat + 64 * l, 192 * 4, 64 * 4, (size_t)P, hipMemcpyDeviceToDevice, st));
             }
             fin = cat + 64 * l;
+            fins = psplit ? cats + 64 * l : nullptr;
             ldin = 192;
         }
         if (m->sf16 && m->opt_fn_maxfuse) {
@@ -374,6 +393,11 @@
             g.ldc = m->emb; g.epi = EPI_LIF_MAX; g.lif = m->p(FN_FINAL_LIF); g.lif_T = m->T;
             g.max_keys = reinterpret_cast<unsigned*>(B1); g.max_m = mp;
             SAPCU_CHECK_HIP(hipMemsetAsync(g.max_keys, 0, (size_t)cb * m->emb * 4, st));
+            if (psplit) {
+                GemmArgs gs = g;
+                gs.a = cats; gs.a_split = 1;
+                if (split_lif_max_on_big_tile(m, gs)) g = gs;
+            }
             SAPCU_TRY(run_gemm(m, g, st));
             SAPCU_TRY(launch_decode_max_keys(g.max_keys, cb * m->emb, pooled, st));
         } else {
@@ -848,6 +872,7 @@
         m->opt_chain_wide = v && strcmp(v, "wide") == 0;
     }
     m->opt_fn_maxfuse = !env_off("SAPCU_FN_MAXFUSE");
+    m->opt_fn_ptsplit = !env_off("SAPCU_FN_PTSPLIT");
     m->opt_fn_fold_out = !env_off("SAPCU_FN_FOLD_OUT");
     for (int l = 0; l < 3; ++l) m->fold_w[l] = m->fold_b[l] = 0;
     m->opt_fd_maxfuse = !env_off("SAPCU_FD_MAXFUSE");
@@ -1015,6 +1040,45 @@
     return SAPCU_OK;
 }
 
+int sapcu_internal_fn_point_route(sapcu_model_t m, int64_t b, int m_pts, int* mask_host) {
+    SAPCU_CHECK_ARG(m && m->kind == SAPCU_KIND_FN && b >= 1 && m_pts >= 1 && mask_host, "fn_point_route: bad argument");
+    const FnPlan pl = fn_plan(m, b, m_pts);
+    int mask = fn_point_split(m) ? 1 : 0;
+    if (mask && m->opt_fn_maxfuse) {
+        GemmArgs g;
+        memset(&g, 0, sizeof(g));
+        g.a = reinterpret_cast<const float*>((uintptr_t)256);
+        g.r = pl.cb * m_pts; g.k = 192; g.lda = 192; g.w = m->p(FN_FINAL_W); g.n = m->emb; g.bias = m->p(FN_FINAL_B);
+        g.ldc = m->emb; g.epi = EPI_LIF_MAX; g.lif = m->p(FN_FINAL_LIF); g.lif_T = m->T;
+        g.max_keys = reinterpret_cast<unsigned*>((uintptr_t)256); g.max_m = m_pts; g.a_split = 1;
+        if (split_lif_max_on_big_tile(m, g)) mask |= 2;
+    }
+    *mask_host = mask;
+    return SAPCU_OK;
+}
+
+int sapcu_internal_gemm_lif_max(const float* a, int64_t r, int k, int lda, const float* w, int n, const float* bias, const float* lif4,
+                                int lif_steps, int max_m, void* keys_ws, float* pooled_out, void* w16_ws, int a_split_rows,
+                                void* stream) {
+    SAPCU_CHECK_ARG(a && w && lif4 && keys_ws && pooled_out && w16_ws && r >= 1 && n >= 1 && k >= 32 && k % 32 == 0 && lda >= k &&
+                        lif_steps >= 1 && max_m >= 1, "gemm_lif_max: bad argument");
+    SAPCU_CHECK_ARG(a_split_rows || k % 64 == 0, "gemm_lif_max: the f32-A kernel steps k by 64");
+    hipStream_t st = (hipStream_t)stream;
+    const int64_t groups = (r + max_m - 1) / max_m;
+    GemmArgs g;
+    memset(&g, 0, sizeof(g));
+    g.a = a; g.r = r; g.k = k; g.lda = lda; g.w = w; g.n = n; g.bias = bias; g.ldc = n;
+    g.epi = EPI_LIF_MAX; g.lif = lif4; g.lif_T = lif_steps; g.max_keys = (unsigned*)keys_ws; g.max_m = max_m;
+    g.a_split = a_split_rows ? 1 : 0;
+    g.w16_hi = (const _Float16*)w16_ws;
+    g.w16_lo = (const _Float16*)w16_ws + (int64_t)n * k;
+    SAPCU_CHECK_ARG(!g.a_split || gemm_sf16_bt_ok(g), "gemm_lif_max: the big-tile kernel does not take this shape");
+    SAPCU_TRY(split_into_ws(w, (int64_t)n * k, w16_ws, g, st));
+    SAPCU_CHECK_HIP(hipMemsetAsync(keys_ws, 0, (size_t)groups * n * 4, st));
+    SAPCU_TRY(g.a_split ? launch_gemm_sf16_bt(g, st) : launch_gemm_sf16(g, st));
+    return launch_decode_max_keys(g.max_keys, groups * n, pooled_out, st);
+}
+
 int sapcu_internal_fold_affine_host(const float* w_out, const float* b_out, const float* w_fc2, const float* b_fc2, int d, int n,
                                     float* w_fold_out, float* b_fold_out) {
     SAPCU_CHECK_ARG(w_out && b_out && w_fc2 && b_fc2 && w_fold_out && b_fold_out && d >= 1 && n >= 1, "fold_affine: bad argument");
diff --git a/c-users-sayakdutta-self-supervised-arbitrary-scale-point-cloud-upsampling-via-snn_amd/csrc/ops.h b/c-users-sayakdutta-self-supervised-arbitrary-scale-point-cloud-upsampling-via-snn_amd/csrc/ops.h
--- a/c-users-sayakdutta-self-supervised-arbitrary-scale-point-cloud-upsampling-via-snn_amd/csrc/ops.h
+++ b/c-users-sayakdutta-self-supervised-arbitrary-scale-point-cloud-upsampling-via-snn_amd/csrc/ops.h
@@ -14,7 +14,7 @@
 int launch_neuron_drive(const float* x, int64_t rows, int ch, int T, const float* md, const float* ta, const float* rd, const float* tb,
                         const float* dT, const float* rh, int pairv, float* so, float* mo, float* to, float* ro, int* gate, hipStream_t st);
 int launch_fn_stem(const float* patch, int64_t rows, const float* w, const float* bias, const float* lif, int T,
-                   float* out, hipStream_t st);
+                   float* out, float* out_split, hipStream_t st);
 int launch_fn_pe1(const float* patch, const int32_t* idx, int64_t rows, int m, int kk, int d, const float* w,
                   const float* bias, const float* lif, int T, float* out, int split, hipStream_t st);
 struct ChainArgs {
diff --git a/c-users-sayakdutta-self-supervised-arbitrary-scale-point-cloud-upsampling-via-snn_amd/csrc/patch_ops.hip b/c-users-sayakdutta-self-supervised-arbitrary-scale-point-cloud-upsampling-via-snn_amd/csrc/patch_ops.hip
--- a/c-users-sayakdutta-self-supervised-arbitrary-scale-point-cloud-upsampling-via-snn_amd/csrc/patch_ops.hip
+++ b/c-users-sayakdutta-self-supervised-arbitrary-scale-point-cloud-upsampling-via-snn_amd/csrc/patch_ops.hip
@@ -310,7 +310,7 @@
 __global__ __launch_bounds__(256) void fn_stem_kernel(const float* __restrict__ patch, int64_t rows,
                                                       const float* __restrict__ w ,
                                                       const float* __restrict__ bias, const float* __restrict__ lif,
-                                                      int T, float* __restrict__ out) {
+                                                      int T, float* __restrict__ out, float* __restrict__ out_split) {
     const int64_t t = (int64_t)blockIdx.x * blockDim.x + threadIdx.x;
     if (t >= rows * 64) return;
     const int c = (int)(t & 63);
@@ -320,14 +320,16 @@
     a = __fmaf_rn(w[c * 3 + 1], y, a);
     a = __fmaf_rn(w[c * 3 + 2], z, a);
     a = __fadd_rn(a, bias[c]);
-    out[t] = lif_selfloop(a, load_lif(lif, 64, c), T);
+    const float v = lif_selfloop(a, load_lif(lif, 64, c), T);
+    out[t] = v;
+    if (out_split) store_split(out_split, r, 64, c, v);
 }
 
 int launch_fn_stem(const float* patch, int64_t rows, const float* w, const float* bias, const float* lif, int T,
-                   float* out, hipStream_t st) {
+                   float* out, float* out_split, hipStream_t st) {
     if (rows == 0) return SAPCU_OK;
     hipLaunchKernelGGL(fn_stem_kernel, dim3((unsigned)((rows * 64 + 255) / 256)), dim3(256), 0, st, patch, rows, w,
-                       bias, lif, T, out);
+                       bias, lif, T, out, out_split);
     SAPCU_CHECK_LAUNCH();
     return SAPCU_OK;
 }
```

Result: no change. 125,800 query-points/s, median of 6 (+0.6%).
